# hsinnan75/Dart

Measured on AMD Instinct MI355X. Metric: M paired-end reads/sec (2x101 bp vs GRCh38-sized index), host to host; records bit-identical to CPU dart, higher is better.
Workload: dtype u64/u8 integer

## Files before the change

### dart_amd/csrc/dg_api.hip

```cpp
#include "../../include/dartgpu.h"
#include "dg_common.h"
#include "dg_fm.h"
#include "dg_seedq.h"
#include "dg_chain.h"
#include "dg_report.h"
#include "dg_pair.h"
#include "dg_reseed.h"
#include "dg_sort.h"
#include "dg_samfmt.h"
#include "dg_bamfmt.h"
#include "dg_bgzf.h"
#include "dg_bgzf_dyn.h"
#include "dg_fastq.h"
#include "dg_trim.h"
#include "dg_inflate.h"
#include "dg_sjtab.h"
#include "dg_bamsort.h"
#include "dg_bamidx.h"
#include "dg_coverage.h"
#include "dg_markdup.h"
#include "dg_umidup.h"
#include "dg_pileup.h"
#include "dg_qc.h"
#include "dg_tags.h"
#include "dg_genecount.h"
#include "dg_rnametrics.h"
#include "dg_txquant.h"
#include <stdio.h>
#include <stdlib.h>
#include <string.h>
#include <string>
#include <algorithm>
#include <vector>
#include <atomic>
#include <mutex>
#include <chrono>
#include <thread>
#include <condition_variable>
#include <fcntl.h>
#include <unistd.h>
#include <sys/stat.h>

static char g_init_error[512] = "";

#define DG_HW_QUEUES_NEED 16
static_assert(DG_HW_QUEUES_NEED <= 32, "more hardware queues than 32 are not asked for");
static char g_hwq_found[24] = "unset";
static int g_hwq_left = DG_HW_QUEUES_NEED;
__attribute__((constructor)) static void dg_default_hw_queues()
{
    const char *v = getenv("GPU_MAX_HW_QUEUES");
    long have = 0;
    if (v) {
        size_t i = 0;
        for (; v[i] && i + 1 < sizeof g_hwq_found; i++) g_hwq_found[i] = (v[i] > ' ' && v[i] < 127 && v[i] != ';' && v[i] != '=') ? v[i] : '?';
        g_hwq_found[i] = 0;
        if (!i) snprintf(g_hwq_found, sizeof g_hwq_found, "empty");
        char *end = nullptr;
        have = strtol(v, &end, 10);
        if (end == v || *end) have = 0; else if (have > 1000000) have = 1000000;
    }
    if (have < DG_HW_QUEUES_NEED) {
        char b[8];
        snprintf(b, sizeof b, "%d", DG_HW_QUEUES_NEED);
        setenv("GPU_MAX_HW_QUEUES", b, 1);
        have = DG_HW_QUEUES_NEED;
    }
    g_hwq_left = (int)have;
}
static std::atomic<int> g_live_ctx[64];
static std::atomic<bool> g_hwq_warned{false};

#include "api_ctx.h"

#define N_TIMERS 20
#define N_TOPS 128
enum { TOP_CIG = 0, TOP_SJ, TOP_JOBS, TOP_REPORT_MAIN, TOP_REPORT_JOBS , TOP_HEAVY_UNITS, TOP_SEED_NEXT, TOP_SEED_HEAVY,
       TOP_WORK = 16, TOP_TICKET_PAIR = 17, TOP_TICKET_EMIT = 18, TOP_RESEED_COUNT = 19 , TOP_RESEED_TICKET = 23 , TOP_TICKET_SEED = 26, TOP_RS_POOL = 27, TOP_RS_OUT = 31,
       TOP_ORDER_INFO = 28 , TOP_CLASS_HIST = 32 , TOP_CLASS_FILL = 64  };

struct IndexShared {
    std::mutex mu;
    std::condition_variable cv;
    DIndex ix{};
    std::atomic<uint32_t> gen{1};
    std::thread aids;
    std::atomic<int> aids_state{0};
    char aids_msg[256] = "";
    bool upload_done = false, upload_ok = false;
    void *d_ktab = nullptr, *d_sa_dense = nullptr;
    std::string report, report_out;
    int device = 0;
    uint32_t *d_chr_name_off = nullptr; char *d_chr_names = nullptr; bool chr_names_set = false; uint64_t chr_names_gen = 0; uint32_t chr_name_max = 0;
    uint32_t *d_gc_chr_first = nullptr, *d_gc_seg_start = nullptr, *d_gc_seg_lab = nullptr; uint32_t gc_n_genes = 0; size_t gc_n_seg = 0; uint64_t gc_gen = 0;
    uint32_t *d_rm_chr_first = nullptr, *d_rm_seg_start = nullptr, *d_rm_seg_cs = nullptr; RmTx *d_rm_tx = nullptr; RmExon *d_rm_ex = nullptr;
    size_t rm_n_seg = 0, rm_n_tx = 0, rm_n_elig = 0; uint64_t rm_gen = 0;
    uint32_t *d_tx_chr_first = nullptr, *d_tx_seg_start = nullptr, *d_tx_seg_ids = nullptr; uint64_t *d_tx_seg_off = nullptr; TxTx *d_tx_tx = nullptr; TxExon *d_tx_ex = nullptr;
    size_t tx_n_seg = 0; uint32_t tx_n_tx = 0; uint64_t tx_gen = 0;
};

struct dg_ctx {
    int device = 0;
    IndexShared *shared_ix = nullptr; uint32_t ix_gen = 0;
    bool owns_index = true;
    hipStream_t stream = nullptr;
    hipEvent_t ev_dl = nullptr, ev_dl_block = nullptr;
    bool dl_on_copy_stream = false;
    int env_copy_stream = 1;
    hipEvent_t ev_wait = nullptr;
    char err[512] = "";
    DIndex ix{};
    DParams pr{};
    void *d_bwt = nullptr, *d_sa = nullptr, *d_pac = nullptr, *d_lockey = nullptr, *d_locchr = nullptr, *d_chroff = nullptr;
    int n_reads = 0, max_rlen = 0;
    size_t seq_bytes = 0;
    bool enc_ready = false;
    DBuf<unsigned char> seq; DBuf<uint32_t> seq_off; DBuf<uint16_t> rlen; DBuf<uint32_t> enc; DBuf<uint32_t> packed_in, nlist_in;
    DBuf<DHit> hits; DBuf<uint32_t> nhits, nseeds, seed_off, ncand, rep_off, tile_sums, tile_read, slow_units;
    DBuf<SKey> seeds; DBuf<DSeed> work; DBuf<DCand> cands; DBuf<DJob> jobs; DBuf<unsigned long long> job_items, job_pool; DBuf<RsChunkOut> job_outs; DBuf<uint32_t> job_pool_next; DBuf<unsigned long long> items; DBuf<uint32_t> hist, heavy; DBuf<DHeavy> seed_heavy; DBuf<int32_t> seed_heavy_sfail; DBuf<int16_t> chain_picks; DBuf<uint8_t> chain_todo;
    DBuf<dg_read_out> reads_out; DBuf<dg_report_out> reports; DBuf<uint32_t> cigpool, cigfinal;
    DBuf<dg_sj_out> sjpool, sjfinal;
    DBuf<dg_read_c> reads_c; DBuf<dg_report_c> reports_c; DBuf<uint32_t> cig_c;
    DBuf<unsigned char> ws;
    DBuf<unsigned long long> scan_state, scan_trace;
    int wall_khz = 100000;
    uint32_t scan_epoch = 0;
    size_t cap_seeds = 0, cap_rep = 0, cap_work = 0, cap_cig = 0;
    struct SharedCaps { std::atomic<size_t> seeds{0}, rep{0}, work{0}, cig{0}; } *shared_caps = nullptr;
    bool owns_shared_caps = false;
    unsigned long long *d_ctr = nullptr; unsigned int *d_tops = nullptr; int *d_err = nullptr; DSizes *d_sizes = nullptr; unsigned int *d_input_bad = nullptr;
    struct HostTail { DSizes sizes; int err; unsigned int input_bad; unsigned int tops[N_TOPS]; unsigned long long ctr[CTR_STRIDE]; __host__ __device__ uint32_t *sizes_words() { return (uint32_t *)&sizes; } } *h_tail = nullptr;
    bool state_zeroed = false;
    size_t used[3] = {0, 0, 0};
    bool enqueued = false;
    hipEvent_t ev[N_TIMERS + 1] = {}; const char *tname[N_TIMERS]; int n_t = 0; float tms[N_TIMERS];
    uint64_t counters[CTR_N];
    uint64_t reruns_capacity = 0, reruns_scan = 0;
    bool want_compact = true, packed_valid = false;
    bool batch_done = false;
    bool no_batch = false;
    SamState sam; FqState fq; TrimState tr; InfState inf; BamState bam; SjState sj; BsState bs; BiState bi; CvState cv; MdState md; UdState ud; PuState pu; QcState qc; TgState tg; GcState gc; RmState rm; TxState tx;
    bool want_full = true, full_valid = false;
    int n_cu = 256, runs_of_last_batch = 0, attempt_no = 0;
    int env_seed_waves = 4, env_bail_trips = 0 , env_report_bpc = 8, env_no_fast = 0, env_seed_legacy = 0, env_seed_slots_lg = 0, env_seed_wgs = 0, env_blocking_sync = 0;
    int env_seed_phases = 0, env_seed_wg_waves = 4, env_seed_partial = 32, env_seed_multi = 4;
    bool seed_qf_used = false;
    int env_scan_mask = 7;
    int env_chain_bpc = 8, env_seedh_bpc = 8, env_reseed_pct = 100;
    int env_rs_chunk = RS_CHUNK_DIAGS, env_rs_inline = RS_ENT_INLINE, env_rs_pool = 0;
    int env_scan_budget = 0;
    ~dg_ctx() {
        for (void *p : {(void *)d_ctr, (void *)d_tops, (void *)d_err, (void *)d_sizes, (void *)d_input_bad}) if (p) (void)hipFree(p);
        if (h_tail) (void)hipHostFree(h_tail);
        for (hipEvent_t e : ev) if (e) (void)hipEventDestroy(e);
        for (hipEvent_t e : {ev_wait, ev_dl, ev_dl_block}) if (e) (void)hipEventDestroy(e);
        if (owns_shared_caps) delete shared_caps;
    }
};

static void read_env(dg_ctx *c)
{
    auto geti = [](const char *k, int dflt) { const char *v = getenv(k); return v ? atoi(v) : dflt; };
    c->env_seed_waves = geti("DG_SEED_WAVES", 4); c->env_bail_trips = geti("DG_SEED_BAIL_TRIPS", 0);
    c->env_seed_legacy = geti("DG_SEED_LEGACY", 0); c->env_seed_slots_lg = geti("DG_SEED_SLOTS_LG", 0); c->env_seed_wgs = geti("DG_SEED_WGS", 0); c->env_blocking_sync = geti("DG_BLOCKING_SYNC", 0);
    c->env_report_bpc = geti("DG_REPORT_BPC", 8); c->env_no_fast = geti("DG_NO_FAST_PAIR", 0);
    c->env_scan_budget = geti("DG_SCAN_POLL_BUDGET", 0); c->env_scan_mask = geti("DG_SCAN_POLL_SCANS", 7);
    c->env_seed_phases = geti("DG_SEED_PHASES", 0); c->env_seed_wg_waves = geti("DG_SEED_WG_WAVES", 4); c->env_seed_partial = geti("DG_SEED_PARTIAL_MIN", 32);
    c->env_copy_stream = geti("DG_COPY_STREAM", 1);
    c->env_chain_bpc = std::max(1, geti("DG_CHAIN_BPC", 8)); c->env_seedh_bpc = std::max(1, geti("DG_SEEDH_BPC", 8)); c->env_reseed_pct = std::max(10, geti("DG_RESEED_PCT", 100));
    c->env_rs_chunk = geti("DG_RS_CHUNK", RS_CHUNK_DIAGS); c->env_rs_chunk = std::min(1 << 24, std::max(RS_SUPER, c->env_rs_chunk / RS_SUPER * RS_SUPER));
    c->env_rs_inline = std::min(RS_ENT_INLINE, std::max(0, geti("DG_RS_ENT_MAX", RS_ENT_INLINE))); c->env_rs_pool = std::max(0, geti("DG_RS_POOL_BLOCKS", 0));
    c->sam.first_cap = (size_t)std::max(0, geti("DG_SAM_TEXT_FIRST_CAP", 0));
    c->bam.first_cap = (size_t)std::max(0, geti("DG_BAM_FIRST_CAP", 0));
    c->bs.first_cap = (size_t)std::max(0, geti("DG_BAMSORT_FIRST_CAP", 0));
    c->md.hash_bits = geti("DG_MARKDUP_HASH_BITS", MD_HASH_BITS); if (c->md.hash_bits < 1 || c->md.hash_bits > MD_HASH_BITS) c->md.hash_bits = MD_HASH_BITS;
    c->qc.max_groups = geti("DG_QC_MAX_GROUPS", QC_GROUPS); if (c->qc.max_groups < 1 || c->qc.max_groups > QC_GROUPS) c->qc.max_groups = QC_GROUPS;
    c->rm.max_groups = geti("DG_RNA_MAX_GROUPS", RM_GROUPS); if (c->rm.max_groups < 1 || c->rm.max_groups > RM_GROUPS) c->rm.max_groups = RM_GROUPS;
    c->tx.hash_bits = geti("DG_TX_HASH_BITS", 64); if (c->tx.hash_bits < 1 || c->tx.hash_bits > 64) c->tx.hash_bits = 64;
    c->env_seed_multi = geti("DG_SEED_MULTI", 4); if (c->env_seed_multi < 0 || c->env_seed_multi > SQF_MULTI_MAX) c->env_seed_multi = SQF_MULTI_MAX;
}

static inline void refresh_index(dg_ctx *c)
{
    IndexShared *sh = c->shared_ix;
    if (sh && c->ix_gen != sh->gen.load(std::memory_order_acquire)) { std::lock_guard<std::mutex> lk(sh->mu); c->ix = sh->ix; c->ix_gen = sh->gen.load(); }
}

static int fail(dg_ctx *c, int code, const char *what, hipError_t e)
{
    snprintf(c ? c->err : g_init_error, 512, "%s: %s", what, e == hipSuccess ? "error" : hipGetErrorString(e));
    return code;
}
#define HIPCHK(call) do { hipError_t _e = (call); if (_e != hipSuccess) return fail(c, DG_ERR_HIP, #call, _e); } while (0)

#define SO_PER 8
__global__ void __launch_bounds__(256)
k_seed_offsets(int n_reads, int paired, const uint32_t *__restrict__ nseeds, uint32_t *__restrict__ seed_off, uint32_t *__restrict__ tile_read, uint32_t n_tile_read,
               uint32_t *__restrict__ heavy_list, unsigned int *n_heavy, uint32_t *total_copy, uint32_t cap, TileScan ts, int *err)
{
    __shared__ unsigned long long s_scan[20];
    __shared__ unsigned int s_tile;
    const unsigned int tile = d_tile_ticket_unless(ts, &s_tile, threadIdx.x == 0 && __hip_atomic_load(err, __ATOMIC_RELAXED, __HIP_MEMORY_SCOPE_AGENT) >= DG_ABORT);
    if (tile == SCAN_LEAVE) return;
    const uint32_t first = tile * (256u * SO_PER) + threadIdx.x * SO_PER;
    uint32_t v[SO_PER], sum = 0;
    if (first + SO_PER <= (uint32_t)n_reads) {
        const uint4 a = *(const uint4 *)(nseeds + first), b = *(const uint4 *)(nseeds + first + 4);
        v[0] = a.x; v[1] = a.y; v[2] = a.z; v[3] = a.w; v[4] = b.x; v[5] = b.y; v[6] = b.z; v[7] = b.w;
    } else {
#pragma unroll
        for (int i = 0; i < SO_PER; i++) v[i] = first + i < (uint32_t)n_reads ? nseeds[first + i] : 0u;
    }
#pragma unroll
    for (int i = 0; i < SO_PER; i++) sum += v[i];
    Triple mine, tot;
    mine.x = sum; mine.y = 0; mine.z = 0; mine.w = 0;
    const Triple inb = d_block_exclusive(mine, tot, s_scan);
    const Triple base = d_tile_exclusive(ts, tile, tot, s_scan + 16, err);
    uint32_t run = base.x + inb.x;
    const int lane = threadIdx.x & 63;
#pragma unroll
    for (int i = 0; i < SO_PER; i++) {
        const uint32_t r = first + i;
        if (r < (uint32_t)n_reads) {
            seed_off[r] = run;
            for (uint32_t t = (run + 63u) >> 6; (t << 6) < run + v[i] && t < n_tile_read; t++) tile_read[t] = r;
        }
        const bool unit_end = paired ? (i & 1) == 1 : true;
        const uint32_t useeds = paired ? ((i & 1) ? v[i - ((i & 1) ? 1 : 0)] + v[i] : 0u) : v[i];
        const bool heavy = unit_end && r < (uint32_t)n_reads && useeds > (uint32_t)UNIT_MAX_SEEDS;
        const unsigned long long m = __ballot(heavy);
        if (m) {
            unsigned int hb = 0;
            const int leader = __ffsll((long long)m) - 1;
            if (lane == leader) hb = atomicAdd(n_heavy, (unsigned int)__popcll(m));
            hb = (unsigned int)__shfl((int)hb, leader, 64);
            if (heavy) heavy_list[hb + (unsigned int)__popcll(m & ((1ull << lane) - 1ull))] = paired ? r >> 1 : r;
        }
        run += v[i];
    }
    if (tile == gridDim.x - 1 && threadIdx.x == 0) {
        const uint32_t total = base.x + tot.x;
        seed_off[n_reads] = total;
        if (total_copy) *total_copy = total;
        if (total > cap) atomicMax(err, DG_E_SEEDS);
    }
}

static std::atomic<uint64_t> g_phase_ns[4];
static void caps_publish(std::atomic<size_t> &a, size_t v) { size_t cur = a.load(); while (cur < v && !a.compare_exchange_weak(cur, v)) { } }
static void caps_adopt(size_t &mine, const std::atomic<size_t> &a) { const size_t v = a.load(); if (v > mine) mine = v; }
static std::mutex g_copy_mu[64];
static hipStream_t g_copy_stream[64][2];
static hipError_t copy_stream(int device, int dir, hipStream_t *out)
{
    hipStream_t &sl = g_copy_stream[device & 63][dir];
    if (!sl) {
        int lo = 0, hi = 0;
        hipError_t e = hipDeviceGetStreamPriorityRange(&lo, &hi);
        if (e == hipSuccess) e = hipStreamCreateWithPriority(&sl, hipStreamNonBlocking, hi);
        if (e != hipSuccess) { sl = nullptr; return e; }
    }
    *out = sl;
    return hipSuccess;
}

static bool host_page_locked(const void *p)
{
    if (!p) return false;
    hipPointerAttribute_t a;
    if (hipPointerGetAttributes(&a, p) != hipSuccess) { (void)hipGetLastError(); return false; }
    return a.type == hipMemoryTypeHost;
}

static hipError_t wait_stream(dg_ctx *c)
{
    if (!c->env_blocking_sync || !c->ev_wait) return hipStreamSynchronize(c->stream);
    const hipError_t e = hipEventRecord(c->ev_wait, c->stream);
    return e != hipSuccess ? e : hipEventSynchronize(c->ev_wait);
}

#ifdef DG_PROFILE_CLASSES
__device__ unsigned long long g_class_cycles[DG_COST_CLASSES + 1], g_class_chunks[DG_COST_CLASSES + 1];
#endif
template <int MINW>
__global__ void __launch_bounds__(64, MINW)
k_report(const DIndex ix, const DParams pr, int n_reads, int paired, const unsigned char *__restrict__ seq,
         const uint32_t *__restrict__ seq_off, const uint16_t *__restrict__ rlen, const uint32_t *__restrict__ seed_off,
         const DJob *__restrict__ jobs, DCand *__restrict__ cands,
         const uint32_t *__restrict__ rep_off, DSeed *__restrict__ work, const unsigned long long *__restrict__ items,
         const uint32_t *__restrict__ n_items_p, dg_report_out *__restrict__ reports, uint32_t *cigpool, uint32_t cigcap,
         unsigned int *tops, unsigned char *ws, const WSLayout L, unsigned long long *ctr, int *err)
{
    const unsigned long long t_wave0 = wall_clock64();
    const int lane = blockIdx.x * blockDim.x + threadIdx.x;
    __shared__ uint32_t lds_pm[64 * PM_LDS_WORDS];
    if (*err >= DG_ABORT) return;
    LaneCtx cx;
#ifdef DG_PROFILE_CLASSES
    __shared__ unsigned long long ph_acc[DG_NCLS * DG_NPHASE], cls_acc[2 * DG_NCLS];
    for (int q = threadIdx.x; q < DG_NCLS * DG_NPHASE; q += 64) ph_acc[q] = 0;
    for (int q = threadIdx.x; q < 2 * DG_NCLS; q += 64) cls_acc[q] = 0;
    __syncthreads();
    cx.ph = ph_acc;
#endif
    cx.lds = lds_pm + (threadIdx.x & 63) * PM_LDS_WORDS;
    cx.ix = &ix; cx.pr = &pr; cx.L = &L;
    cx.ws = ws + (size_t)lane * L.stride;
    cx.n_nw = cx.nw_cells = cx.n_reseed = cx.reseed_w = 0;
    const unsigned int lo = 0u, hi = *n_items_p;
    unsigned int *next = tops + TOP_REPORT_MAIN;
    while (true) {
        unsigned int ticket = 0;
        if ((threadIdx.x & 63) == 0) ticket = atomicAdd(next, 1u);
        ticket = (unsigned int)__shfl((int)ticket, 0, 64);
        const unsigned int base = lo + ticket * 64u;
        if (base >= hi) break;
        const unsigned int idx = base + (threadIdx.x & 63);
        const bool valid = idx < hi;
        const unsigned long long item = valid ? items[idx] : 0ull;
        const int r = (int)(item >> 32);
        const uint32_t ci = (uint32_t)item, rep_i = valid ? rep_off[r] + (ci - seed_off[r]) : 0u;
        DRead rd;
        rd.sub_score = 0; rd.mis_num = 0; rd.mapq = 0;
        cx.seq = seq + seq_off[r]; cx.rlen = rlen[r];
#ifdef DG_PROFILE_CLASSES
        const long long t_begin = clock64();
        cx.cls = (int)(cands[(uint32_t)items[base]].final_n & 31); cx.t_last = t_begin;
#endif
        d_gen_mapping_report(cx, valid, paired ? (r & 1) == 0 : true, rd, cands + ci, valid ? 1 : 0, jobs, work,
                             reports + rep_i, rep_i, cigpool, tops + 0, cigcap, err, 0, 1, true);
#ifdef DG_PROFILE_CLASSES
        if ((threadIdx.x & 63) == 0) { cls_acc[cx.cls] += (unsigned long long)(clock64() - t_begin); cls_acc[DG_NCLS + cx.cls] += 1ull; }
#endif
    }
#ifdef DG_PROFILE_CLASSES
    __syncthreads();
    for (int q = threadIdx.x; q < DG_NCLS * DG_NPHASE; q += 64) if (ph_acc[q]) atomicAdd(&g_phase[q / DG_NPHASE][q % DG_NPHASE], ph_acc[q]);
    if (threadIdx.x < DG_NCLS && cls_acc[DG_NCLS + threadIdx.x]) { atomicAdd(&g_class_cycles[threadIdx.x], cls_acc[threadIdx.x]); atomicAdd(&g_class_chunks[threadIdx.x], cls_acc[DG_NCLS + threadIdx.x]); }
#endif
    d_wave_add(ctr + CTR_NW, cx.n_nw);
    d_wave_add(ctr + CTR_NWCELLS, cx.nw_cells);
    d_wave_add(ctr + CTR_RESEED, cx.n_reseed);
    d_wave_add(ctr + CTR_RESEEDW, cx.reseed_w);
    d_wave_resident(ctr, CTR_WT_REPORT, t_wave0);
}

__global__ void __launch_bounds__(256)
k_finalize(const DIndex ix, const DParams pr, int paired, const uint32_t *__restrict__ slow_units, const DSizes *__restrict__ sizes,
           const uint32_t *__restrict__ seed_off, const DCand *__restrict__ cands, const uint32_t *__restrict__ ncand, const uint32_t *__restrict__ rep_off, const DSeed *__restrict__ work,
           dg_read_out *__restrict__ rout, dg_report_out *__restrict__ reports, dg_sj_out *sjpool, uint32_t sjcap, unsigned int *tops, int *err)
{
    if (*err >= DG_ABORT) return;
    const unsigned int n_units = sizes->n_slow_units;
    for (unsigned int it = blockIdx.x * blockDim.x + threadIdx.x; it < n_units; it += gridDim.x * blockDim.x) {
        const int u = (int)slow_units[it];
        const int nm = paired ? 2 : 1;
        DRead rd[2];
        dg_read_out o[2];
        RepMem<dg_report_out> rp[2];
        for (int m = 0; m < nm; m++) {
            const int r = paired ? 2 * u + m : u;
            const int nc = (int)ncand[r];
            dg_report_out *rep = reports + rep_off[r];
            rd[m].score = 0; rd[m].sub_score = 0; rd[m].mis_num = 0; rd[m].mapq = 0; rd[m].iBest = 0; rd[m].CanNum = nc > 0 ? nc : 1;
            for (int i = 0; i < nc; i++) {
                const int aln = rep[i].aln_score, mis_num = rep[i].flag;
                if (mis_num) rep[i].flag = 0;
                if (aln <= 0) continue;
                if (aln > rd[m].score) { rd[m].iBest = i; rd[m].mis_num = mis_num; rd[m].sub_score = rd[m].score; rd[m].score = aln; }
                else if (aln == rd[m].score) rd[m].sub_score = rd[m].score;
            }
            o[m].score = rd[m].score; o[m].sub_score = rd[m].sub_score; o[m].mis_num = rd[m].mis_num; o[m].mapq = 0;
            o[m].n_rep = rd[m].CanNum; o[m].best = rd[m].iBest; o[m].rep_off = (int32_t)rep_off[r]; o[m].sj_off = 0; o[m].n_sj = 0;
            rp[m].p = rep;
        }
        if (paired) {
            d_settle_pair(pr, rd[0], rp[0], rd[1], rp[1]);
            d_flag_pair(rd[0], rp[0], rd[1], rp[1]);
        } else d_flag_single(rd[0], rp[0]);
        for (int m = 0; m < nm; m++) {
            const int r = paired ? 2 * u + m : u;
            d_mapq(rd[m], rp[m]);
            o[m].score = rd[m].score; o[m].mapq = rd[m].mapq; o[m].best = rd[m].iBest;
            if (ncand[r] > 0 && (rd[m].mapq == 50 || (pr.all_sj && rd[m].score > 0)))
                d_collect_sj(ix, pr, cands[seed_off[r] + rd[m].iBest], work, r, sjpool, tops + TOP_SJ, sjcap, o[m].sj_off, o[m].n_sj, err);
            rout[r] = o[m];
        }
    }
}

__global__ void __launch_bounds__(256)
k_emit_slow(int paired, const uint32_t *__restrict__ slow_units, DSizes *sizes, dg_read_out *__restrict__ rout, dg_report_out *__restrict__ reports,
            const uint32_t *__restrict__ cigpool, uint32_t *__restrict__ cigfinal, uint32_t cap_cig, const dg_sj_out *__restrict__ sjpool, dg_sj_out *__restrict__ sjfinal,
            TileScan ts, int *err, const uint16_t *__restrict__ rlen, const CompactOut co)
{
    __shared__ unsigned long long s_scan[20];
    __shared__ unsigned int s_tile;
    bool leave = false;
    if (threadIdx.x == 0) { const int e0 = __hip_atomic_load(err, __ATOMIC_RELAXED, __HIP_MEMORY_SCOPE_AGENT); leave = e0 >= DG_ABORT && e0 != DG_E_CIGFINAL; }
    const unsigned int tile = d_tile_ticket_unless(ts, &s_tile, leave);
    if (tile == SCAN_LEAVE) return;
    const unsigned int n_items = sizes->n_slow_units * (paired ? 2u : 1u);
    if (tile > 0 && tile * 256u >= n_items) return;
    const unsigned int it = tile * 256u + threadIdx.x;
    const bool on = it < n_items;
    const int r = on ? (paired ? (int)(2u * slow_units[it >> 1] + (it & 1u)) : (int)slow_units[it]) : 0;
    dg_read_out o;
    o.n_rep = 0; o.rep_off = 0; o.n_sj = 0; o.sj_off = 0;
    if (on) o = rout[r];
    uint32_t ncig = 0, ncigc = 0;
    const uint32_t full_match = on ? (uint32_t)rlen[r] << 4 : 0u;
    for (int i = 0; i < (on ? o.n_rep : 0); i++) {
        const dg_report_out &rp = reports[o.rep_off + i];
        ncig += rp.n_cigar;
        if (co.reads) ncigc += (rp.n_cigar == 1u && cigpool[rp.cigar_off] == full_match) ? 0u : rp.n_cigar;
    }
    Triple mine, tot;
    mine.x = ncig; mine.y = on ? (uint32_t)o.n_sj : 0u; mine.z = 0; mine.w = ncigc;
    const Triple inb = d_block_exclusive(mine, tot, s_scan);
    const Triple base = d_tile_exclusive(ts, tile, tot, s_scan + 16, err);
    const uint32_t cig_fast = sizes->cig_fast, cigc_fast = sizes->pad[2];
    if (on) {
        uint32_t dst = cig_fast + base.x + inb.x, dstc = cigc_fast + base.w + inb.w;
        bool fits = true;
        if ((uint64_t)dst + ncig > cap_cig) atomicMax(err, DG_E_CIGFINAL);
        else for (int i = 0; i < o.n_rep; i++) {
            dg_report_out &rp = reports[o.rep_off + i];
            const uint32_t m = rp.n_cigar, src = rp.cigar_off;
            const bool plain = m == 1u && cigpool[src] == full_match;
            for (uint32_t k = 0; k < m; k++) cigfinal[dst + k] = cigpool[src + k];
            if (co.reads) {
                if (!plain) { for (uint32_t k = 0; k < m; k++) co.cigar[dstc + k] = cigpool[src + k]; dstc += m; }
                dg_report_c q; fits = d_compact_report(rp, plain, true, q) && fits; co.reports[o.rep_off + i] = q;
            }
            rp.cigar_off = dst; dst += m;
        }
        if (o.n_sj > 0) {
            const uint32_t sd = base.y + inb.y;
            for (int k = 0; k < o.n_sj; k++) sjfinal[sd + k] = sjpool[o.sj_off + k];
            rout[r].sj_off = (int32_t)sd;
        }
        if (co.reads) { dg_read_c oc; fits = d_compact_read(o, oc) && fits; co.reads[r] = oc; if (!fits) *co.bad = 1u; }
    }
    const unsigned int last = n_items ? (n_items - 1u) / 256u : 0u;
    if (tile == last && threadIdx.x == 0) { sizes->total_cig = cig_fast + base.x + tot.x; sizes->total_sj = base.y + tot.y; sizes->pad[0] = cigc_fast + base.w + tot.w; }
}

extern "C" void dg_params_default(dg_params *p)
{
    p->max_gaps = 5; p->max_dup = 100; p->max_intron = 500000; p->min_intron = 5;
    p->max_mismatch = 0; p->multi_hit = 0; p->all_sj = 0; p->paired = 0;
}

static void set_params(dg_ctx *c, const dg_params *p)
{
    c->pr.max_gaps = p->max_gaps; c->pr.max_dup = p->max_dup; c->pr.max_intron = p->max_intron; c->pr.min_intron = p->min_intron;
    c->pr.max_mismatch = p->max_mismatch; c->pr.multi_hit = p->multi_hit; c->pr.all_sj = p->all_sj; c->pr.paired = p->paired;
}

extern "C" int dg_set_params(dg_ctx *c, const dg_params *p)
{
    if (!c || !p) return DG_ERR_ARG;
    set_params(c, p);
    read_env(c);
    return DG_OK;
}

extern "C" int dg_device_count(void)
{
// ... 602 lines not shown
    if (trimmed) {
        const TrimInfo &ti = *c->tr.info.h;
        memcpy(c->tr.stats, ti.stats, sizeof c->tr.stats); c->tr.ms = c->tr.ev.ms(0, 1);
        n_reads = ti.n_kept;
        if (n_reads_out) *n_reads_out = (int)n_reads;
    }
    if (!keep) return DG_OK;
    c->n_reads = (int)n_reads; c->max_rlen = (int)fi.max_rlen; c->seq_bytes = (size_t)fi.total[0];
    c->fq.hdr_bytes = (size_t)fi.total[1]; c->fq.qual_bytes = (size_t)fi.total[2]; c->fq.valid = true;
    return DG_OK;
}

static void fq_forget_batch(dg_ctx *c)
{
    c->n_reads = 0; c->max_rlen = 0; c->seq_bytes = 0; c->enc_ready = false; c->enqueued = false; c->batch_done = false; c->sj.batch_counted = false; c->gc.batch_counted = false; c->tx.batch_counted = false; c->sam.valid = false; c->bam.valid = false; c->bam.rec_valid = false; c->bam.rec_stored = false; c->fq.valid = false;
    c->fq.hdr_bytes = c->fq.qual_bytes = 0; c->fq.ms = 0.f;
    memset(c->tr.stats, 0, sizeof c->tr.stats); c->tr.ms = 0.f; c->tr.enqueued = false;
    c->no_batch = false; c->inf.valid = false; c->fq.tail_valid = false; c->fq.tail_n[0] = c->fq.tail_n[1] = 0;
}

extern "C" int dg_batch_upload_fastq(dg_ctx *c, const dg_fastq_text *in, int *n_reads_out)
{
    if (!c) return DG_ERR_ARG;
    if (n_reads_out) *n_reads_out = 0;
    fq_forget_batch(c);
    if (!in) { snprintf(c->err, 512, "dg_batch_upload_fastq: the input is NULL"); return DG_ERR_ARG; }
    const size_t n1 = in->text1 ? in->n1 : 0, n2 = in->text2 ? in->n2 : 0;
    const bool two = in->text2 != nullptr && in->n2 > 0;
    if ((in->n1 && !in->text1) || in->max_reads < 0) { snprintf(c->err, 512, "dg_batch_upload_fastq: text1 is NULL or max_reads is negative"); return DG_ERR_ARG; }
    if (n1 >= 0xFFFFFF00ull || n2 >= 0xFFFFFF00ull) { snprintf(c->err, 512, "dg_batch_upload_fastq: a text must be smaller than 2^32 - 256 bytes"); return DG_ERR_ARG; }
    if (n1 == 0 && !two) { c->fq.valid = true; return DG_OK; }
    HIPCHK(hipSetDevice(c->device));
    FqPlan p;
    p.n[0] = n1; p.n[1] = n2; p.two = two; p.max_reads = (size_t)in->max_reads;
    { const int rc = fq_reserve(c, p); if (rc) return rc; }
    if (n1) HIPCHK(hipMemcpyAsync(c->fq.text.p, in->text1, n1, hipMemcpyHostToDevice, c->stream));
    if (n2) HIPCHK(hipMemcpyAsync(c->fq.text.p + p.off2, in->text2, n2, hipMemcpyHostToDevice, c->stream));
    HIPCHK(hipEventRecord(c->fq.ev[0], c->stream));
    { const int rc = fq_enqueue(c, p, in->rc_odd_reads, false, false, true); if (rc) return rc; }
    HIPCHK(wait_stream(c));
    return fq_finish(c, "dg_batch_upload_fastq", in->max_reads, n_reads_out, true);
}

static int inf_enqueue_copies(dg_ctx *c, const std::vector<InfBlock> &tab, const void *src1, size_t n1, const void *src2, size_t n2, size_t in_off2)
{
    HIPCHK(c->inf.in.ensure(std::max(n1, in_off2 + n2) + 8)); HIPCHK(c->inf.tab.ensure(tab.size() + 1)); HIPCHK(c->inf.status.ensure(tab.size() + 1));
    if (n1) HIPCHK(hipMemcpyAsync(c->inf.in.p, src1, n1, hipMemcpyHostToDevice, c->stream));
    if (n2) HIPCHK(hipMemcpyAsync(c->inf.in.p + in_off2, src2, n2, hipMemcpyHostToDevice, c->stream));
    if (!tab.empty()) HIPCHK(hipMemcpyAsync(c->inf.tab.p, tab.data(), tab.size() * sizeof(InfBlock), hipMemcpyHostToDevice, c->stream));
    HIPCHK(hipMemsetAsync(c->inf.verdict.d, 0xff, 8, c->stream));
    return DG_OK;
}
static int inf_enqueue_kernel(dg_ctx *c, size_t n_blocks, unsigned char *d_out)
{
    if (n_blocks) k_bgzf_inflate<<<(unsigned)((n_blocks + INF_WAVES - 1) / INF_WAVES), 64 * INF_WAVES, 0, c->stream>>>(c->inf.in.p, c->inf.tab.p, (uint32_t)n_blocks, d_out, c->inf.status.p, c->inf.verdict.d);
    HIPCHK(hipGetLastError());
    HIPCHK(c->inf.verdict.fetch(c->stream));
    return DG_OK;
}

extern "C" int dg_inflate_granules(int out[2])
{
    if (!out) return DG_ERR_ARG;
    out[0] = INF_WAVES; out[1] = (int)INF_ROUND;
    return DG_OK;
}

extern "C" int dg_bgzf_inflate(dg_ctx *c, const void *host_bytes, size_t n, size_t *n_out, size_t *n_blocks, float *device_ms)
{
    if (!c) return DG_ERR_ARG;
    if (n_out) *n_out = 0;
    if (n_blocks) *n_blocks = 0;
    if (device_ms) *device_ms = 0.f;
    c->inf.valid = false; c->inf.bytes = 0;
    if (n == 0) { c->inf.valid = true; return DG_OK; }
    if (!host_bytes) { snprintf(c->err, 512, "dg_bgzf_inflate: the input is NULL"); return DG_ERR_ARG; }
    std::vector<InfBlock> tab;
    size_t total = 0, bad = 0;
    if (const char *why = inf_walk_members((const unsigned char *)host_bytes, n, 0, 0, tab, &total, &bad)) { snprintf(c->err, 512, "dg_bgzf_inflate: block %zu: %s", bad, why); return DG_ERR_ARG; }
    if (tab.size() > 0x7fffffffull) { snprintf(c->err, 512, "dg_bgzf_inflate: %zu blocks are more than one call takes", tab.size()); return DG_ERR_ARG; }
    HIPCHK(hipSetDevice(c->device));
    HIPCHK(c->inf.ready());
    HIPCHK(c->inf.out.ensure(total + 32));
    { const int rc = inf_enqueue_copies(c, tab, host_bytes, n, nullptr, 0, 0); if (rc) return rc; }
    HIPCHK(hipEventRecord(c->inf.ev[0], c->stream));
    { const int rc = inf_enqueue_kernel(c, tab.size(), c->inf.out.p); if (rc) return rc; }
    HIPCHK(hipEventRecord(c->inf.ev[1], c->stream));
    HIPCHK(wait_stream(c));
    const float ms = c->inf.ev.ms(0, 1);
    if (device_ms) *device_ms = ms;
    if (n_blocks) *n_blocks = tab.size();
    const unsigned long long v = *c->inf.verdict.h;
    if (v != ~0ull) { snprintf(c->err, 512, "dg_bgzf_inflate: block %llu: %s", v >> 8, inf_rule((uint32_t)(v & 0xffu))); return DG_ERR_ARG; }
    c->inf.valid = true; c->inf.bytes = total;
    if (n_out) *n_out = total;
    return DG_OK;
}

extern "C" int dg_inflate_download(dg_ctx *c, void *out, size_t cap)
{
    if (!c) return DG_ERR_ARG;
    if (!c->inf.valid) { snprintf(c->err, 512, "dg_inflate_download: no inflated bytes (dg_bgzf_inflate first)"); return DG_ERR_ARG; }
    if (cap < c->inf.bytes) { snprintf(c->err, 512, "dg_inflate_download: output capacity too small: %zu bytes of %zu", cap, c->inf.bytes); return DG_ERR_CAPACITY; }
    if (c->inf.bytes == 0) return DG_OK;
    if (!out) return DG_ERR_ARG;
    HIPCHK(hipSetDevice(c->device));
    HIPCHK(hipMemcpyAsync(out, c->inf.out.p, c->inf.bytes, hipMemcpyDeviceToHost, c->stream));
    HIPCHK(wait_stream(c));
    return DG_OK;
}

extern "C" int dg_inflate_device(dg_ctx *c, void **ptr, size_t *n_out)
{
    if (!c || !ptr || !n_out) return DG_ERR_ARG;
    if (!c->inf.valid) { snprintf(c->err, 512, "dg_inflate_device: no inflated bytes (dg_bgzf_inflate first)"); return DG_ERR_ARG; }
    *ptr = c->inf.bytes ? c->inf.out.p : nullptr; *n_out = c->inf.bytes;
    return DG_OK;
}

extern "C" int dg_batch_upload_fastq_bgzf(dg_ctx *c, const dg_fastq_bgzf *in, uint32_t flags, int *n_reads_out, size_t tail[2], uint64_t *n_unlike)
{
    static const char *fn = "dg_batch_upload_fastq_bgzf";
    if (!c) return DG_ERR_ARG;
    if (n_reads_out) *n_reads_out = 0;
    if (tail) tail[0] = tail[1] = 0;
    if (n_unlike) *n_unlike = 0;
    fq_forget_batch(c);
    if (!in) { snprintf(c->err, 512, "%s: the input is NULL", fn); return DG_ERR_ARG; }
    if (flags & ~DG_FQ_CHECK_ONLY) { snprintf(c->err, 512, "%s: unknown flag bits 0x%x", fn, flags & ~DG_FQ_CHECK_ONLY); return DG_ERR_ARG; }
    const bool check_only = (flags & DG_FQ_CHECK_ONLY) != 0, two = in->blocks2 != nullptr || in->head2 != nullptr, last = in->last != 0;
    if ((in->n_head1 && !in->head1) || (in->n_blocks1 && !in->blocks1) || (in->n_head2 && !in->head2) || (in->n_blocks2 && !in->blocks2) || in->max_reads < 0) {
        snprintf(c->err, 512, "%s: a length without its pointer, or max_reads is negative", fn); return DG_ERR_ARG;
    }
    const size_t nh[2] = { in->head1 ? in->n_head1 : 0, in->head2 ? in->n_head2 : 0 }, nb[2] = { in->blocks1 ? in->n_blocks1 : 0, two && in->blocks2 ? in->n_blocks2 : 0 };
    const unsigned char *src[2] = { (const unsigned char *)in->blocks1, (const unsigned char *)in->blocks2 };
    const size_t in_off2 = (nb[0] + 255) & ~(size_t)255;
    std::vector<InfBlock> tab;
    size_t n_inf[2] = {0, 0}, first2 = 0;
    for (int f = 0; f < (two ? 2 : 1); f++) {
        size_t bad = 0;
        if (f) first2 = tab.size();
        if (const char *why = inf_walk_members(src[f], nb[f], f ? in_off2 : 0, nh[f], tab, &n_inf[f], &bad)) { snprintf(c->err, 512, "%s: text %d block %zu: %s", fn, f + 1, bad, why); return DG_ERR_ARG; }
        if (nh[f] + n_inf[f] >= 0xFFFFFF00ull) { snprintf(c->err, 512, "%s: a text must be smaller than 2^32 - 256 bytes", fn); return DG_ERR_ARG; }
    }
    if (!two) first2 = tab.size();
    if (tab.size() > 0x7fffffffull) { snprintf(c->err, 512, "%s: %zu blocks are more than one call takes", fn, tab.size()); return DG_ERR_ARG; }
    FqPlan p;
    p.n[0] = nh[0] + n_inf[0]; p.n[1] = nh[1] + n_inf[1]; p.two = two; p.max_reads = (size_t)in->max_reads;
    if (p.n[0] == 0 && p.n[1] == 0) { c->fq.valid = !check_only; c->no_batch = check_only; c->fq.tail_valid = true; return DG_OK; }
    HIPCHK(hipSetDevice(c->device));
    HIPCHK(c->inf.ready());
    { const int rc = fq_reserve(c, p); if (rc) return rc; }
    for (size_t k = first2; k < tab.size(); k++) tab[k].out_off += p.off2;
    c->fq.tail_off2 = (p.n[0] + 255) & ~(size_t)255;
    HIPCHK(c->fq.tail.ensure(c->fq.tail_off2 + p.n[1] + 16));
    { const int rc = inf_enqueue_copies(c, tab, src[0], nb[0], src[1], nb[1], in_off2); if (rc) return rc; }
    if (nh[0]) HIPCHK(hipMemcpyAsync(c->fq.text.p, in->head1, nh[0], hipMemcpyHostToDevice, c->stream));
    if (nh[1]) HIPCHK(hipMemcpyAsync(c->fq.text.p + p.off2, in->head2, nh[1], hipMemcpyHostToDevice, c->stream));
    HIPCHK(hipEventRecord(c->fq.ev[0], c->stream));
    { const int rc = inf_enqueue_kernel(c, tab.size(), c->fq.text.p); if (rc) return rc; }
    { const int rc = fq_enqueue(c, p, in->rc_odd_reads, !last, true, !check_only); if (rc) return rc; }
    HIPCHK(wait_stream(c));
    const unsigned long long v = *c->inf.verdict.h;
    if (v != ~0ull) {
        const size_t k = (size_t)(v >> 8);
        snprintf(c->err, 512, "%s: text %d block %zu: %s", fn, k >= first2 ? 2 : 1, k >= first2 ? k - first2 : k, inf_rule((uint32_t)(v & 0xffu)));
        return DG_ERR_ARG;
    }
    const FqInfo &fi = *c->fq.info.h;
    if (n_unlike) *n_unlike = fi.n_unlike;
    const int rc = fq_finish(c, fn, in->max_reads, n_reads_out, !check_only);
    if (fi.status == FQ_OK || fi.status == FQ_E_EMPTY || fi.status == FQ_E_LONG || fi.status == FQ_E_OFFSETS) {
        c->fq.tail_n[0] = p.n[0] - fi.tail_at[0]; c->fq.tail_n[1] = two ? p.n[1] - fi.tail_at[1] : 0;
        c->fq.tail_valid = true;
        if (tail) { tail[0] = c->fq.tail_n[0]; tail[1] = c->fq.tail_n[1]; }
    }
    if (rc == DG_OK && check_only) c->no_batch = true;
    return rc;
}

extern "C" int dg_batch_download_fastq_tail(dg_ctx *c, char *tail1, size_t cap1, char *tail2, size_t cap2)
{
    if (!c) return DG_ERR_ARG;
    if (!c->fq.tail_valid) { snprintf(c->err, 512, "dg_batch_download_fastq_tail: no tails (dg_batch_upload_fastq_bgzf first)"); return DG_ERR_ARG; }
    if (cap1 < c->fq.tail_n[0] || cap2 < c->fq.tail_n[1]) { snprintf(c->err, 512, "dg_batch_download_fastq_tail: output capacity too small (need %zu %zu)", c->fq.tail_n[0], c->fq.tail_n[1]); return DG_ERR_CAPACITY; }
    if ((c->fq.tail_n[0] && !tail1) || (c->fq.tail_n[1] && !tail2)) return DG_ERR_ARG;
    if (!c->fq.tail_n[0] && !c->fq.tail_n[1]) return DG_OK;
    HIPCHK(hipSetDevice(c->device));
    if (c->fq.tail_n[0]) HIPCHK(hipMemcpyAsync(tail1, c->fq.tail.p, c->fq.tail_n[0], hipMemcpyDeviceToHost, c->stream));
    if (c->fq.tail_n[1]) HIPCHK(hipMemcpyAsync(tail2, c->fq.tail.p + c->fq.tail_off2, c->fq.tail_n[1], hipMemcpyDeviceToHost, c->stream));
    HIPCHK(wait_stream(c));
    return DG_OK;
}

extern "C" int dg_batch_fastq_device_ms(dg_ctx *c, float *ms)
{
    if (!c || !ms) return DG_ERR_ARG;
    *ms = c->fq.ms;
    return DG_OK;
}

extern "C" int dg_set_trim(dg_ctx *c, const dg_trim *t)
{
    if (!c) return DG_ERR_ARG;
    if (!t) { c->tr.on = false; return DG_OK; }
    if (t->flags & ~DG_TRIM_PAIRS) { snprintf(c->err, 512, "dg_set_trim: unknown flag bits 0x%x", t->flags & ~DG_TRIM_PAIRS); return DG_ERR_ARG; }
    if (t->min_len == 0 || t->min_overlap == 0) { snprintf(c->err, 512, "dg_set_trim: min_len and min_overlap must be at least 1"); return DG_ERR_ARG; }
    if (t->max_err_permille > 1000u) { snprintf(c->err, 512, "dg_set_trim: max_err_permille is %u, above 1000", t->max_err_permille); return DG_ERR_ARG; }
    if (t->poly_mask & ~15u) { snprintf(c->err, 512, "dg_set_trim: poly_mask 0x%x has a bit above 3", t->poly_mask); return DG_ERR_ARG; }
    if (t->qual3 > TR_QUAL_MAX || t->qual5 > TR_QUAL_MAX || t->qual_base > TR_QUAL_MAX) { snprintf(c->err, 512, "dg_set_trim: qual3, qual5 and qual_base must not exceed %u", TR_QUAL_MAX); return DG_ERR_ARG; }
    TrimPar par = {};
    for (int i = 0; i < 2; i++) {
        if (t->n_adapter[i] > 64u) { snprintf(c->err, 512, "dg_set_trim: adapter %d has %u bases, more than 64", i, t->n_adapter[i]); return DG_ERR_ARG; }
        for (uint32_t j = 0; j < t->n_adapter[i]; j++) {
            const char b = t->adapter[i][j];
            if (b != 'A' && b != 'C' && b != 'G' && b != 'T') { snprintf(c->err, 512, "dg_set_trim: adapter %d has a byte outside ACGT at %u", i, j); return DG_ERR_ARG; }
            par.acode[i][j >> 5] |= (uint64_t)trim_code(b) << (2u * (j & 31u));
        }
        par.alen[i] = t->n_adapter[i];
    }
    par.flags = t->flags; par.qual3 = t->qual3; par.qual5 = t->qual5; par.qual_base = t->qual_base; par.min_overlap = t->min_overlap; par.max_err_permille = t->max_err_permille;
    par.poly_mask = t->poly_mask; par.poly_min = t->poly_min; par.min_len = t->min_len;
    c->tr.par = par; c->tr.on = true;
    return DG_OK;
}

extern "C" int dg_set_umi(dg_ctx *c, const dg_umi *u)
{
    if (!c) return DG_ERR_ARG;
    if (!u) { c->tr.umi_on = false; return DG_OK; }
    if (u->flags & ~DG_UMI_PAIRS) { snprintf(c->err, 512, "dg_set_umi: unknown flag bits 0x%x", u->flags & ~DG_UMI_PAIRS); return DG_ERR_ARG; }
    if ((uint64_t)u->len[0] + u->len[1] == 0 || (uint64_t)u->len[0] + u->len[1] > UD_MAX_LEN) { snprintf(c->err, 512, "dg_set_umi: the two lengths together are %llu, not 1..%d", (unsigned long long)u->len[0] + u->len[1], UD_MAX_LEN); return DG_ERR_ARG; }
    for (int m = 0; m < 2; m++)
        if ((uint64_t)u->len[m] + u->skip[m] > (uint64_t)DG_MAX_RLEN) { snprintf(c->err, 512, "dg_set_umi: len[%d] + skip[%d] is %llu, above %d", m, m, (unsigned long long)u->len[m] + u->skip[m], DG_MAX_RLEN); return DG_ERR_ARG; }
    if (u->sep == 0 || u->sep == ' ' || u->sep == '\t' || u->sep == '/' || ud_code((unsigned char)u->sep)) { snprintf(c->err, 512, "dg_set_umi: the separator 0x%02x is NUL, a blank, a tab, '/' or one of ACGTN+-", (unsigned char)u->sep); return DG_ERR_ARG; }
    c->tr.umi = *u; c->tr.umi_on = true;
    return DG_OK;
}

extern "C" int dg_batch_trim_stats(dg_ctx *c, uint64_t stats[16], float *device_ms)
{
    if (!c || !stats) return DG_ERR_ARG;
    memcpy(stats, c->tr.stats, sizeof c->tr.stats);
    if (device_ms) *device_ms = c->tr.ms;
    return DG_OK;
}

extern "C" int dg_trim_granules(int out[2])
{
    if (!out) return DG_ERR_ARG;
    out[0] = FQ_THREADS; out[1] = 64;
    return DG_OK;
}

extern "C" int dg_batch_download_reads(dg_ctx *c, uint32_t *seq_off, uint16_t *rlen, char *seq, uint32_t *hdr_off, char *hdr, uint32_t *qual_off, char *qual,
                                       const size_t caps[3], size_t used[3])
{
    if (!c || !caps || !used) return DG_ERR_ARG;
    if (!c->fq.valid) { snprintf(c->err, 512, "dg_batch_download_reads: the context's last upload was not dg_batch_upload_fastq"); return DG_ERR_ARG; }
    used[0] = c->seq_bytes; used[1] = c->fq.hdr_bytes; used[2] = c->fq.qual_bytes;
    if (caps[0] < used[0] || caps[1] < used[1] || caps[2] < used[2]) { snprintf(c->err, 512, "dg_batch_download_reads: output capacity too small (need %zu %zu %zu)", used[0], used[1], used[2]); return DG_ERR_CAPACITY; }
    const size_t n = (size_t)c->n_reads;
    if (n == 0) { if (hdr_off) hdr_off[0] = 0; if (qual_off) qual_off[0] = 0; return DG_OK; }
    if (!seq_off || !rlen || !hdr_off || !qual_off || (used[0] && !seq) || (used[1] && !hdr) || (used[2] && !qual)) return DG_ERR_ARG;
    HIPCHK(hipSetDevice(c->device));
    HIPCHK(hipMemcpyAsync(seq_off, c->seq_off.p, n * 4, hipMemcpyDeviceToHost, c->stream));
    HIPCHK(hipMemcpyAsync(rlen, c->rlen.p, n * 2, hipMemcpyDeviceToHost, c->stream));
    HIPCHK(hipMemcpyAsync(hdr_off, c->fq.hdr_off.p, (n + 1) * 4, hipMemcpyDeviceToHost, c->stream));
    HIPCHK(hipMemcpyAsync(qual_off, c->fq.qual_off.p, (n + 1) * 4, hipMemcpyDeviceToHost, c->stream));
    if (used[0]) HIPCHK(hipMemcpyAsync(seq, c->seq.p, used[0], hipMemcpyDeviceToHost, c->stream));
    if (used[1]) HIPCHK(hipMemcpyAsync(hdr, c->fq.hdr.p, used[1], hipMemcpyDeviceToHost, c->stream));
    if (used[2]) HIPCHK(hipMemcpyAsync(qual, c->fq.qual.p, used[2], hipMemcpyDeviceToHost, c->stream));
    HIPCHK(wait_stream(c));
    return DG_OK;
}

extern "C" void *dg_host_alloc(size_t bytes)
{
    void *p = nullptr;
    return hipHostMalloc(&p, bytes ? bytes : 1, hipHostMallocDefault) == hipSuccess ? p : nullptr;
}
extern "C" void dg_host_free(void *p) { if (p) (void)hipHostFree(p); }

static WSLayout make_ws_layout(int R)
{
    WSLayout L;
    auto al = [](uint32_t x) { return (x + 15u) & ~15u; };
    uint32_t o = 0;
    const uint32_t nmax = 2u * (uint32_t)R + 32u;
    L.max_rlen = (uint32_t)R;
    L.cig_off = o; L.cig_cap = 4u * (uint32_t)R + 64u; o = al(o + L.cig_cap * 4u);
    L.nwbits_off = o; L.nwbits_words = ((uint32_t)R + 1u) * ((nmax + 7u) / 8u); o = al(o + L.nwbits_words * 4u);
    L.rows_off = o; L.row_cap = (uint32_t)R + 8u; o = al(o + 2u * L.row_cap * 4u);
    L.str_off = o; L.str_cap = al(3u * (uint32_t)R + 64u); o = al(o + 6u * L.str_cap);
    L.kmer_off = o; L.kmer_cap = (uint32_t)R + 8u > 48u ? (uint32_t)R + 8u : 48u; o = al(o + L.kmer_cap * 8u);
    uint32_t rd = 64; while (rd < (uint32_t)R + 1u) rd <<= 1;
    L.ring_diag = rd; L.ring_words = ((uint32_t)R + 64u) / 64u; L.ring_off = o; o = al(o + rd * L.ring_words * 8u);
    L.stride = (o + 255u) & ~255u;
    return L;
}

#define DG_MAX_DEVICES 64
static std::mutex g_lds_mu;
static size_t g_lds_set[2][DG_MAX_DEVICES];
static hipError_t raise_dynamic_lds(const void *fn, int which, int device, size_t lds)
{
    std::lock_guard<std::mutex> lk(g_lds_mu);
    size_t &cur = g_lds_set[which][device & (DG_MAX_DEVICES - 1)];
    if (lds <= cur) return hipSuccess;
    const hipError_t e = hipFuncSetAttribute(fn, hipFuncAttributeMaxDynamicSharedMemorySize, (int)lds);
    if (e == hipSuccess) cur = lds;
    return e;
}

static hipError_t launch_seed(dg_ctx *c, int n, int H, hipEvent_t after_encode = nullptr)
{
    const int W = 2 * ((c->max_rlen + 15) / 16 > 0 ? (c->max_rlen + 15) / 16 : 1);
    hipError_t e = c->enc.ensure((size_t)W * n + 16);
    if (e != hipSuccess) return e;
    int lg = 0;
    while ((1 << lg) < W / 2) lg++;
    if (!c->enc_ready) k_encode<<<(unsigned)((((size_t)n << lg) + 255) / 256), 256, 0, c->stream>>>(c->seq.p, c->seq_off.p, c->rlen.p, n, W, lg, c->enc.p);
    if (after_encode) { e = hipEventRecord(after_encode, c->stream); if (e != hipSuccess) return e; }
    if ((e = c->seed_heavy.ensure((size_t)n + 16)) != hipSuccess) return e;
    unsigned blocks = (unsigned)c->n_cu * (unsigned)c->env_seed_waves;
    if ((size_t)blocks * 64 > (size_t)n) blocks = (unsigned)((n + 63) / 64);
    const bool use_qf = !c->env_seed_legacy && !c->env_seed_phases && W <= 62 && c->pr.max_dup <= 30000;
    const int bail_trips = c->env_bail_trips > 0 ? c->env_bail_trips : (use_qf ? 64 : 128);
    unsigned int *tops = c->d_tops;
    c->seed_qf_used = false;
    if (use_qf) {
        int lg = c->env_seed_slots_lg >= 6 && c->env_seed_slots_lg <= 11 ? c->env_seed_slots_lg : 9;
        int nw = c->env_seed_wg_waves >= 1 && c->env_seed_wg_waves <= 8 ? c->env_seed_wg_waves : 4;
        while (lg > 6 && sqf_lds_bytes(lg, W, nw) > (size_t)156 * 1024) lg--;
        if (c->env_seed_slots_lg == 0) while (lg > 6 && sqf_lds_bytes(lg, W, nw) > (size_t)80 * 1024) lg--;
        const size_t lds = sqf_lds_bytes(lg, W, nw);
        if ((e = raise_dynamic_lds((const void *)k_seed_qf, 0, c->device, lds)) != hipSuccess) return e;
        unsigned per_cu = (unsigned)(((size_t)160 * 1024) / lds);
        if (per_cu * (unsigned)nw > 16u) per_cu = 16u / (unsigned)nw;
        if (per_cu > 2u) per_cu = 2u;
        if (per_cu < 1u) per_cu = 1u;
        if (c->env_seed_wgs > 0) per_cu = (unsigned)c->env_seed_wgs;
        unsigned wgs = (unsigned)c->n_cu * per_cu;
        const unsigned need = (unsigned)(((size_t)n + ((size_t)1 << lg) - 1) >> lg);
        if (wgs > need) wgs = need;
        c->seed_qf_used = true;
        k_seed_qf<<<wgs, nw * 64, lds, c->stream>>>(c->ix, c->pr, c->enc.p, c->rlen.p, n, W, H, lg, c->hits.p, c->nhits.p, c->nseeds.p, tops + TOP_SEED_NEXT,
                                                    c->seed_heavy.p, tops + TOP_SEED_HEAVY, c->d_ctr, bail_trips, c->env_seed_partial, c->env_seed_multi, c->d_err, bail_trips);
    } else
    if (!c->env_seed_legacy && W <= 62) {
        int lg = c->env_seed_slots_lg >= 6 && c->env_seed_slots_lg <= 10 ? c->env_seed_slots_lg : 9;
        while (lg > 6 && sq_lds_bytes(lg, W) > (size_t)80 * 1024) lg--;
        const size_t lds = sq_lds_bytes(lg, W);
        if ((e = raise_dynamic_lds((const void *)k_seed_q, 1, c->device, lds)) != hipSuccess) return e;
        unsigned per_cu = (unsigned)(((size_t)160 * 1024) / lds);
        if (per_cu > 4u) per_cu = 4u;
        if (c->env_seed_wgs > 0) per_cu = (unsigned)c->env_seed_wgs;
        unsigned wgs = (unsigned)c->n_cu * per_cu;
        const unsigned need = (unsigned)(((size_t)n + ((size_t)1 << lg) - 1) >> lg);
        if (wgs > need) wgs = need;
        k_seed_q<<<wgs, SQ_THREADS, lds, c->stream>>>(c->ix, c->pr, c->enc.p, c->rlen.p, n, W, H, lg, c->hits.p, c->nhits.p, c->nseeds.p, tops + TOP_SEED_NEXT,
                                                      c->seed_heavy.p, tops + TOP_SEED_HEAVY, c->d_ctr, bail_trips, c->d_err);
    } else
    if (W <= 78) k_seed<true><<<blocks, 64, ((size_t)2 * W * 64 + 64) * 4, c->stream>>>(c->ix, c->pr, c->enc.p, c->rlen.p, n, W, H, c->hits.p, c->nhits.p, c->nseeds.p, tops + TOP_SEED_NEXT, c->seed_heavy.p, tops + TOP_SEED_HEAVY, c->d_ctr, bail_trips);
    else k_seed<false><<<blocks, 64, 0, c->stream>>>(c->ix, c->pr, c->enc.p, c->rlen.p, n, W, H, c->hits.p, c->nhits.p, c->nseeds.p, tops + TOP_SEED_NEXT, c->seed_heavy.p, tops + TOP_SEED_HEAVY, c->d_ctr, bail_trips);
    if ((e = c->seed_heavy_sfail.ensure((size_t)n + 16)) != hipSuccess) return e;
    k_seed_heavy_walk<<<(unsigned)c->n_cu * 8u, 64, 0, c->stream>>>(c->ix, c->pr, c->enc.p, c->rlen.p, W, c->seed_heavy.p, tops + TOP_SEED_HEAVY, c->seed_heavy_sfail.p, c->d_ctr);
    k_seed_heavy<<<(unsigned)c->n_cu * (unsigned)c->env_seedh_bpc, 64, (size_t)W * 4 + 16, c->stream>>>(c->ix, c->pr, c->enc.p, c->rlen.p, W, H, c->hits.p, c->nhits.p, c->nseeds.p, c->seed_heavy.p, tops + TOP_SEED_HEAVY, c->seed_heavy_sfail.p, c->d_ctr);
    return hipGetLastError();
}

static TileScan make_tile_scan(dg_ctx *c, size_t first_tile, unsigned int *ticket, int which )
{
    TileScan ts;
    ts.w = c->scan_state.p + SCAN_WORDS * first_tile; ts.ticket = ticket; ts.epoch = c->scan_epoch;
    ts.budget = (c->env_scan_budget > 0 && c->attempt_no == 0 && (c->env_scan_mask & which)) ? (uint32_t)c->env_scan_budget : 0u;
    ts.dbg = c->d_sizes->scan_dbg;
    ts.ticks = (unsigned long long)c->wall_khz * 2000ull;
    ts.trace = c->scan_trace.p ? c->scan_trace.p + SCAN_TRACE_WORDS * first_tile : nullptr;
    return ts;
}

#define TICK(name) do { if (c->n_t < N_TIMERS) { c->tname[c->n_t] = name; HIPCHK(hipEventRecord(c->ev[c->n_t + 1], c->stream)); c->n_t++; } } while (0)

static int enqueue_seeding(dg_ctx *c, int n, int H, bool timed, bool paired_units)
{
    HIPCHK(c->hits.ensure((size_t)n * H)); HIPCHK(c->nhits.ensure(n)); HIPCHK(c->nseeds.ensure(n)); HIPCHK(c->seed_off.ensure((size_t)n + 1));
    if (c->shared_caps) caps_adopt(c->cap_seeds, c->shared_caps->seeds);
    if (c->cap_seeds < (size_t)n * 3 + 1024) c->cap_seeds = (size_t)n * 3 + 1024;
    HIPCHK(c->seeds.ensure(c->cap_seeds + 1)); HIPCHK(c->cands.ensure(c->cap_seeds + 1)); HIPCHK(c->tile_read.ensure(c->cap_seeds / 64 + 16));
    if (timed) c->tname[c->n_t] = "k_encode";
    HIPCHK(launch_seed(c, n, H, timed ? c->ev[c->n_t + 1] : nullptr));
    if (timed) { c->n_t++; TICK("k_seed"); }
    {
        const int paired = (paired_units && (n % 2 == 0)) ? 1 : 0;
        HIPCHK(c->heavy.ensure((size_t)n + 16));
        const TileScan ts_seed = make_tile_scan(c, 0, c->d_tops + TOP_TICKET_SEED, 1);
        k_seed_offsets<<<(unsigned)((n + 256 * SO_PER - 1) / (256 * SO_PER)), 256, 0, c->stream>>>(n, paired, c->nseeds.p, c->seed_off.p, c->tile_read.p, (uint32_t)c->tile_read.cap,
                                                                                                 c->heavy.p, c->d_tops + TOP_HEAVY_UNITS, &c->d_sizes->total_seeds, (uint32_t)c->cap_seeds, ts_seed, c->d_err);
        HIPCHK(hipGetLastError());
    }
    if (timed) TICK("seed_offsets");
    k_locate<<<(unsigned)((c->cap_seeds + 255) / 256), 256, 0, c->stream>>>(c->ix, n, H, c->hits.p, c->tile_read.p, c->seed_off.p, c->seeds.p, c->d_ctr, c->d_err);
    HIPCHK(hipGetLastError());
    if (timed) TICK("k_locate");
    return DG_OK;
}

__global__ void __launch_bounds__(256)
k_batch_begin(unsigned long long *ctr, unsigned int *tops, int *err, DSizes *sizes)
{
    for (int i = threadIdx.x; i < CTR_STRIPES * CTR_STRIDE; i += 256) ctr[i] = 0ull;
    if (threadIdx.x < N_TOPS) tops[threadIdx.x] = 0u;
    if (threadIdx.x < (int)(sizeof(DSizes) / 4)) ((uint32_t *)sizes)[threadIdx.x] = 0u;
    if (threadIdx.x == 0) *err = 0;
}

static size_t scan_tiles_seed(int n_reads) { return (size_t)(n_reads + 256 * SO_PER - 1) / (256 * SO_PER) + 1; }
static size_t scan_tiles_pair(int n_units) { return (size_t)(n_units + PU_THREADS - 1) / PU_THREADS + 1; }

__global__ void __launch_bounds__(256)
k_batch_end(DSizes *__restrict__ sizes, int *__restrict__ err, unsigned int *__restrict__ tops, unsigned long long *__restrict__ ctr, dg_ctx::HostTail *out)
{
    const int t = threadIdx.x;
    if (t < (int)(sizeof(DSizes) / 4)) { out->sizes_words()[t] = ((const uint32_t *)sizes)[t]; ((uint32_t *)sizes)[t] = 0u; }
    if (t < N_TOPS) { out->tops[t] = tops[t]; tops[t] = 0u; }
    if (t == 0) { out->err = *err; *err = 0; }
    if (t < CTR_STRIDE) {
        const bool is_max = t == CTR_MAXTRIPS || t == CTR_WTRIPS_MAX;
        unsigned long long v = 0;
        for (int s_ = 0; s_ < CTR_STRIPES; s_++) { const unsigned long long x = ctr[s_ * CTR_STRIDE + t]; ctr[s_ * CTR_STRIDE + t] = 0ull; v = is_max ? (x > v ? x : v) : v + x; }
        out->ctr[t] = v;
    }
}

static int zero_batch_state(dg_ctx *c, int n_reads, int n_units)
{
    if (!c->state_zeroed) {
        k_batch_begin<<<1, 256, 0, c->stream>>>(c->d_ctr, c->d_tops, c->d_err, c->d_sizes);
        HIPCHK(hipGetLastError());
    }
    c->state_zeroed = false;
    const size_t tiles2 = (size_t)(2 * n_units + 255) / 256 + 1;
    const size_t words = SCAN_WORDS * (scan_tiles_seed(n_reads) + scan_tiles_pair(n_units) + tiles2);
    if (words > c->scan_state.cap) {
        HIPCHK(c->scan_state.ensure(words));
        HIPCHK(hipMemsetAsync(c->scan_state.p, 0, c->scan_state.cap * 8, c->stream));
        static_assert(SCAN_TRACE_WORDS == SCAN_WORDS, "the trace array is sized like the state array");
        HIPCHK(c->scan_trace.ensure(c->scan_state.cap));
        HIPCHK(hipMemsetAsync(c->scan_trace.p, 0, c->scan_trace.cap * 8, c->stream));
    }
    c->scan_epoch = (c->scan_epoch + 1u) & 0x3FFFFFFFu;
    if (c->scan_epoch == 0) c->scan_epoch = 1;
    return DG_OK;
}


static int enqueue_run(dg_ctx *c)
{
    const int n = c->n_reads;
    const int paired = (c->pr.paired && (n % 2 == 0)) ? 1 : 0;
    const int n_units = paired ? n / 2 : n;
    refresh_index(c);
    c->n_t = 0;
    const int H = c->max_rlen / 16 + 1;
    const uint32_t nb = (uint32_t)((n + 255) / 256);
    { const int zr = zero_batch_state(c, n, n_units); if (zr) return zr; }
    HIPCHK(hipEventRecord(c->ev[0], c->stream));
    { const int rc = enqueue_seeding(c, n, H, true, c->pr.paired != 0); if (rc) return rc; }

    if (c->shared_caps) { caps_adopt(c->cap_rep, c->shared_caps->rep); caps_adopt(c->cap_cig, c->shared_caps->cig); caps_adopt(c->cap_work, c->shared_caps->work); }
    if (c->cap_rep < (size_t)n + (size_t)n / 4 + 1024) c->cap_rep = (size_t)n + (size_t)n / 4 + 1024;
    if (c->cap_cig < 3 * c->cap_rep) c->cap_cig = 3 * c->cap_rep;
    if (c->cap_work < (size_t)n * 8 + 65536) c->cap_work = (size_t)n * 8 + 65536;
    const size_t cigcap = (size_t)n * 48 + c->cap_rep * (16 + CIG_SLOT) + 4096, sjcap = (size_t)n * 4 + 1024;
    HIPCHK(c->ncand.ensure(n)); HIPCHK(c->rep_off.ensure((size_t)n + 1)); HIPCHK(c->reads_out.ensure(n));
    HIPCHK(c->heavy.ensure((size_t)n_units + 16)); HIPCHK(c->slow_units.ensure((size_t)n_units + 16));
    HIPCHK(c->reports.ensure(c->cap_rep + 1)); HIPCHK(c->work.ensure(c->cap_work + 16)); HIPCHK(c->jobs.ensure(c->cap_seeds + 16));
    const uint32_t rs_out_cap = (uint32_t)std::max<size_t>(16384, (size_t)n / 8), rs_list_cap = (uint32_t)std::min<size_t>(c->jobs.cap + rs_out_cap, 0xFFFFFFF0u);
    HIPCHK(c->job_outs.ensure(rs_out_cap)); HIPCHK(c->job_items.ensure(3 * (size_t)rs_list_cap + 16));
    const uint32_t rs_pool_cap = (uint32_t)std::max<size_t>(16384, (size_t)n / 32);
    HIPCHK(c->job_pool.ensure((size_t)rs_pool_cap * 64)); HIPCHK(c->job_pool_next.ensure(rs_pool_cap));
    HIPCHK(c->cigpool.ensure(cigcap)); HIPCHK(c->cigfinal.ensure(c->cap_cig + 16)); HIPCHK(c->sjpool.ensure(sjcap)); HIPCHK(c->sjfinal.ensure(sjcap));
    HIPCHK(c->items.ensure(c->cap_seeds + 16));
    unsigned int *tops = c->d_tops;

    HIPCHK(c->chain_picks.ensure(c->cap_seeds + 16)); HIPCHK(c->chain_todo.ensure((size_t)n_units + 16));
    k_chain_heavy<<<c->n_cu * c->env_chain_bpc, 64, 0, c->stream>>>(c->ix, c->pr, n_units, paired, c->rlen.p, c->seed_off.p, c->seeds.p, c->cands.p, c->ncand.p,
                                                     c->heavy.p, tops + TOP_HEAVY_UNITS, c->chain_picks.p, c->chain_todo.p, c->d_ctr, c->d_err);
    k_chain_rules<<<c->n_cu * 4, 64, 0, c->stream>>>(paired, c->seed_off.p, c->cands.p, c->ncand.p, c->heavy.p, tops + TOP_HEAVY_UNITS, c->chain_picks.p, c->chain_todo.p, c->d_err);
    HIPCHK(hipGetLastError());
#ifdef DG_PROFILE_CLASSES
    {
        unsigned long long v[3], z = 0;
        HIPCHK(hipStreamSynchronize(c->stream));
        HIPCHK(hipMemcpyFromSymbol(&v[0], HIP_SYMBOL(g_chain_max), 8)); HIPCHK(hipMemcpyFromSymbol(&v[1], HIP_SYMBOL(g_chain_units), 8)); HIPCHK(hipMemcpyFromSymbol(&v[2], HIP_SYMBOL(g_chain_cycles), 8));
        HIPCHK(hipMemcpyToSymbol(HIP_SYMBOL(g_chain_max), &z, 8)); HIPCHK(hipMemcpyToSymbol(HIP_SYMBOL(g_chain_units), &z, 8)); HIPCHK(hipMemcpyToSymbol(HIP_SYMBOL(g_chain_cycles), &z, 8));
        fprintf(stderr, "[chain_heavy] units %llu  mean cycles %llu  max cycles %llu (seeds %llu/%llu cands %llu/%llu)\n", v[1], v[1] ? v[2] / v[1] : 0, v[0] >> 40,
                (v[0] >> 30) & 1023, (v[0] >> 20) & 1023, (v[0] >> 10) & 1023, v[0] & 1023);
    }
#endif
    TICK("k_chain_heavy");
    const size_t tiles_s = scan_tiles_seed(n), tiles = scan_tiles_pair(n_units);
    const TileScan ts_pair = make_tile_scan(c, tiles_s, tops + TOP_TICKET_PAIR, 2), ts_emit = make_tile_scan(c, tiles_s + tiles, tops + TOP_TICKET_EMIT, 4);
    const int try_fast = (c->env_no_fast || c->ix.n_chr > 0xFFFF) ? 0 : 1;
    CompactOut co{nullptr, nullptr, nullptr, nullptr};
    if (c->want_compact) {
        HIPCHK(c->reads_c.ensure((size_t)n + 1)); HIPCHK(c->reports_c.ensure(c->cap_rep + 1)); HIPCHK(c->cig_c.ensure(c->cap_cig + 16));
        co = CompactOut{c->reads_c.p, c->reports_c.p, c->cig_c.p, &c->d_sizes->pad[1]};
    }
    const int W2p = (c->max_rlen + 15) / 16 > 0 ? (c->max_rlen + 15) / 16 : 1;
    const bool packed_pair = c->enc_ready;
    auto launch_pair = [&](auto kernel) {
        kernel<<<(unsigned)((n_units + PU_THREADS - 1) / PU_THREADS), PU_THREADS, 0, c->stream>>>(
            c->ix, c->pr, n_units, paired, try_fast, (c->want_full || !c->want_compact) ? 0 : 2, c->seq.p, c->seq_off.p, c->enc.p, W2p, c->rlen.p, c->seed_off.p, c->seeds.p, c->cands.p, c->ncand.p, c->rep_off.p,
            c->slow_units.p, c->reads_out.p, c->reports.p, c->cigfinal.p, (uint32_t)c->cap_rep, (uint32_t)c->cap_cig, ts_pair, c->d_sizes, tops + TOP_CIG, c->d_ctr, c->d_err, co);
    };
    if (packed_pair) launch_pair(k_pair<true>); else launch_pair(k_pair<false>);
    HIPCHK(hipGetLastError());
    TICK("k_pair");

    const WSLayout L = make_ws_layout(c->max_rlen < 32 ? 32 : c->max_rlen);
    int blocks = c->n_cu * c->env_report_bpc;
    if ((size_t)blocks * 64 > (size_t)n) blocks = (n + 63) / 64;
    {
        const size_t budget = (size_t)12 << 30, per_block = (size_t)64 * L.stride;
        if ((size_t)blocks * per_block > budget) blocks = (int)(budget / per_block);
        if (blocks < 1) blocks = 1;
    }
    HIPCHK(c->ws.ensure((size_t)blocks * 64 * L.stride));
    unsigned slow_grid = (unsigned)c->n_cu * 4u;
    if ((size_t)slow_grid * 256 > (size_t)n) slow_grid = nb;
    k_prep<dg_report_out><<<slow_grid, 256, 0, c->stream>>>(c->pr, paired, c->slow_units.p, c->d_sizes, c->seed_off.p, c->seeds.p, c->cands.p, c->ncand.p, c->work.p, tops + TOP_WORK,
                                             (uint32_t)c->cap_work, c->jobs.p, tops + TOP_JOBS, (uint32_t)c->jobs.cap, c->d_err, c->rlen.p, c->rep_off.p, c->reports.p, tops + TOP_CLASS_HIST,
                                             packed_pair ? c->enc.p : nullptr, W2p, c->seq.p);
    HIPCHK(hipGetLastError());
    TICK("k_prep");
    const uint32_t jobcap = (uint32_t)c->jobs.cap;
    const RsPool rs_pool{c->job_pool.p, c->job_pool_next.p, tops + TOP_RS_POOL, c->env_rs_pool > 0 ? std::min<uint32_t>((uint32_t)c->env_rs_pool, rs_pool_cap) : rs_pool_cap};
    const int rs_gap_max = c->max_rlen - 32, rs_need = rs_gap_max >= 8 ? (rs_gap_max - 8) / 64 + 1 : 1;
    const RsOrder rs_order{c->jobs.p, tops + TOP_JOBS, jobcap, c->job_items.p, rs_list_cap, rs_out_cap, rs_need <= 1 ? 1 : (rs_need <= 2 ? 2 : 4), (uint32_t)c->env_rs_chunk, tops + TOP_RESEED_COUNT, tops + TOP_RS_OUT};
    k_order<<<slow_grid, 256, 0, c->stream>>>(paired, c->slow_units.p, c->d_sizes, c->seed_off.p, c->cands.p, c->ncand.p, tops + TOP_CLASS_HIST, tops + TOP_CLASS_FILL, c->items.p, tops + TOP_ORDER_INFO, rs_order, c->d_err);
    HIPCHK(hipGetLastError());
    TICK("order");
    k_reseed<1><<<c->n_cu * 10 * c->env_reseed_pct / 100, 64, 0, c->stream>>>(c->ix, c->seq.p, c->seq_off.p, c->jobs.p, c->job_items.p, tops + TOP_RESEED_COUNT, tops + TOP_RESEED_COUNT + 3, tops + TOP_RESEED_TICKET, c->job_outs.p, rs_pool, c->env_rs_inline, c->d_ctr, c->d_err);
    if (rs_need > 1) k_reseed<2><<<c->n_cu * 6 * c->env_reseed_pct / 100, 64, 0, c->stream>>>(c->ix, c->seq.p, c->seq_off.p, c->jobs.p, c->job_items.p + rs_list_cap, tops + TOP_RESEED_COUNT + 1, tops + TOP_RESEED_COUNT + 3, tops + TOP_RESEED_TICKET + 1, c->job_outs.p, rs_pool, c->env_rs_inline, c->d_ctr, c->d_err);
    if (rs_need > 2) k_reseed<4><<<c->n_cu * 4 * c->env_reseed_pct / 100, 64, 0, c->stream>>>(c->ix, c->seq.p, c->seq_off.p, c->jobs.p, c->job_items.p + 2 * (size_t)rs_list_cap, tops + TOP_RESEED_COUNT + 2, tops + TOP_RESEED_COUNT + 3, tops + TOP_RESEED_TICKET + 2, c->job_outs.p, rs_pool, c->env_rs_inline, c->d_ctr, c->d_err);
    HIPCHK(hipGetLastError());
    TICK("k_reseed");
    const uint32_t *n_items_p = tops + TOP_ORDER_INFO + 1;
    k_report<2><<<blocks, 64, 0, c->stream>>>(c->ix, c->pr, n, paired, c->seq.p, c->seq_off.p, c->rlen.p, c->seed_off.p, c->jobs.p, c->cands.p,
                                               c->rep_off.p, c->work.p, c->items.p, n_items_p, c->reports.p, c->cigpool.p,
                                               (uint32_t)cigcap, tops, c->ws.p, L, c->d_ctr, c->d_err);
    HIPCHK(hipGetLastError());
#ifdef DG_PROFILE_CLASSES
    {
        unsigned long long cyc[DG_COST_CLASSES + 1], cnt[DG_COST_CLASSES + 1], z[DG_COST_CLASSES + 1] = {0};
        HIPCHK(hipStreamSynchronize(c->stream));
        HIPCHK(hipMemcpyFromSymbol(cyc, HIP_SYMBOL(g_class_cycles), sizeof cyc)); HIPCHK(hipMemcpyFromSymbol(cnt, HIP_SYMBOL(g_class_chunks), sizeof cnt));
        HIPCHK(hipMemcpyToSymbol(HIP_SYMBOL(g_class_cycles), z, sizeof z)); HIPCHK(hipMemcpyToSymbol(HIP_SYMBOL(g_class_chunks), z, sizeof z));
        unsigned long long tot = 0; for (int k = 0; k <= DG_COST_CLASSES; k++) tot += cyc[k];
        unsigned long long ph[DG_NCLS][DG_NPHASE], zp[DG_NCLS][DG_NPHASE] = {{0}};
        HIPCHK(hipMemcpyFromSymbol(ph, HIP_SYMBOL(g_phase), sizeof ph)); HIPCHK(hipMemcpyToSymbol(HIP_SYMBOL(g_phase), zp, sizeof zp));
        for (int k = 0; k < DG_COST_CLASSES; k++) if (cnt[k]) {
            fprintf(stderr, "[class %2d] chunks %7llu  cycles/chunk %8llu  share %5.1f %%  phases/chunk:", k, cnt[k], cyc[k] / cnt[k], 100.0 * cyc[k] / (tot ? tot : 1));
            for (int q = 0; q < DG_NPHASE; q++) fprintf(stderr, " %llu", ph[k][q] / cnt[k]);
            fprintf(stderr, "\n");
        }
    }
#endif
    TICK("k_report");
    k_finalize<<<slow_grid, 256, 0, c->stream>>>(c->ix, c->pr, paired, c->slow_units.p, c->d_sizes, c->seed_off.p, c->cands.p, c->ncand.p, c->rep_off.p, c->work.p,
                                                 c->reads_out.p, c->reports.p, c->sjpool.p, (uint32_t)sjcap, tops, c->d_err);
    k_emit_slow<<<(unsigned)((n + 255) / 256), 256, 0, c->stream>>>(paired, c->slow_units.p, c->d_sizes, c->reads_out.p, c->reports.p, c->cigpool.p, c->cigfinal.p,
                                                                    (uint32_t)c->cap_cig, c->sjpool.p, c->sjfinal.p, ts_emit, c->d_err, c->rlen.p, co);
    HIPCHK(hipGetLastError());
    TICK("k_finalize");
    k_batch_end<<<1, 256, 0, c->stream>>>(c->d_sizes, c->d_err, c->d_tops, c->d_ctr, c->h_tail);
    HIPCHK(hipGetLastError());
    c->state_zeroed = true;
    TICK("tail");
    c->enqueued = true;
    return DG_OK;
}

static int finish_run(dg_ctx *c, size_t used[3])
{
    c->runs_of_last_batch = 0;
    for (int attempt = 0; attempt < 6; attempt++) {
        c->runs_of_last_batch++;
        HIPCHK(wait_stream(c));
        if (c->enc_ready && c->h_tail->input_bad) { snprintf(c->err, 512, "packed batch: the N list holds a position outside the batch"); c->enqueued = false; return DG_ERR_ARG; }
        const DSizes &sz = c->h_tail->sizes;
        const int derr = c->h_tail->err;
        if (derr < DG_ABORT) break;
        auto grow = [](size_t need) { return need + need / 4 + 1024; };
        if (derr == DG_E_SEEDS) c->cap_seeds = grow(sz.total_seeds);
        else if (derr == DG_E_REPORTS) {
            c->cap_rep = std::max(grow(sz.total_rep), 2 * c->cap_rep);
            if (c->cap_cig < 3 * c->cap_rep) c->cap_cig = 3 * c->cap_rep;
        }
        else if (derr == DG_E_WORK) c->cap_work = grow(c->h_tail->tops[TOP_WORK]);
        else if (derr == DG_E_CIGFINAL) c->cap_cig = grow(sz.total_cig > 2 * c->cap_cig ? sz.total_cig : 2 * c->cap_cig);
        if (c->shared_caps) { caps_publish(c->shared_caps->seeds, c->cap_seeds); caps_publish(c->shared_caps->rep, c->cap_rep); caps_publish(c->shared_caps->work, c->cap_work); caps_publish(c->shared_caps->cig, c->cap_cig); }
        if (derr == DG_E_SEEDS || derr == DG_E_REPORTS || derr == DG_E_WORK || derr == DG_E_CIGFINAL) {  }
        else if ((derr == DG_E_SCAN || derr == DG_E_SEEDQ) && attempt < 5) {
            c->reruns_scan++;
            const unsigned long long *d = sz.scan_dbg;
            const double tick_ms = 1.0 / (double)c->wall_khz;
            const bool same_epoch = (d[8] >> 32) == d[5];
            snprintf(c->err, 512, "batch run again (device status %d): look-back of tile %llu gave up on tile %lld after %llu polls / %.1f ms (lane %llu, epoch %llu): words %016llx %016llx %016llx; "
                     "stuck tile's trace: epoch %llu%s HW_ID %08llx (wave %llu simd %llu cu %llu sh %llu se %llu) XCC %llu, ticket %.3f ms before the give-up, own totals %s, prefix %s",
                     derr, d[0] ? d[0] - 1 : 0ull, (long long)d[1], d[6], (double)(d[12] - d[13]) * tick_ms, d[7], d[5], d[2], d[3], d[4],
                     d[8] >> 32, same_epoch ? "" : " (NOT this run's: it never took its ticket here)", d[8] & 0xFFFFFFFFull, d[8] & 15, (d[8] >> 4) & 3, (d[8] >> 8) & 15, (d[8] >> 12) & 1, (d[8] >> 13) & 7, d[11] >> 56,
                     (double)(d[12] - d[9]) * tick_ms, d[10] ? "published" : "NOT published", (d[11] & 0x00FFFFFFFFFFFFFFull) ? "published" : "NOT published");
            if (!c->env_scan_budget) fprintf(stderr, "[libdartgpu] %s\n", c->err);
        }
        else { snprintf(c->err, 512, "device-side scan did not complete (status %d)", derr); return DG_ERR_INTERNAL; }
        if (attempt == 5) { snprintf(c->err, 512, "buffer capacities did not converge (status %d)", derr); return DG_ERR_INTERNAL; }
        if (derr != DG_E_SCAN && derr != DG_E_SEEDQ) c->reruns_capacity++;
        c->attempt_no = attempt + 1;
        const int rc = enqueue_run(c);
        if (rc) return rc;
    }
    c->enqueued = false;
    for (int i = 0; i < c->n_t; i++) { float ms = 0; (void)hipEventElapsedTime(&ms, c->ev[i], c->ev[i + 1]); c->tms[i] = ms; }
    static_assert(CTR_N <= CTR_STRIDE, "the work counters fill one stripe");
    for (int k = 0; k < CTR_N; k++) c->counters[k] = c->h_tail->ctr[k];
    if (c->seed_qf_used) {
        c->counters[CTR_STEPS_ACT] += c->counters[CTR_SQ_LANES + SQ_STEP]; c->counters[CTR_BLOCKS_ACT] += c->counters[CTR_SQ_LANES + SQ_STEP];
        c->counters[CTR_KTAB] += c->counters[CTR_SQ_LANES + SQ_BEGIN]; c->counters[CTR_DIRECT] += c->counters[CTR_SQ_LANES + SQ_LOC] + c->counters[CTR_SQ_LANES + SQ_CMP];
    }
    const DSizes &sz = c->h_tail->sizes;
    c->counters[CTR_SEEDS] = sz.total_seeds;
    const int derr = c->h_tail->err;
    if (derr) { snprintf(c->err, 512, "device pool exhausted (%s)", derr == DG_E_CIGAR ? "cigar" : (derr == DG_E_SJ ? "splice junction" : "reseed jobs")); return DG_ERR_INTERNAL; }
    c->used[0] = sz.total_rep; c->used[1] = sz.total_cig; c->used[2] = sz.total_sj;
    c->packed_valid = c->want_compact; c->full_valid = c->want_full || !c->want_compact;
    if (used) { used[0] = c->used[0]; used[1] = c->used[1]; used[2] = c->used[2]; }
    return DG_OK;
}

extern "C" int dg_batch_run(dg_ctx *c, size_t used[3])
{
    if (!c) return DG_ERR_ARG;
    if (c->no_batch) { snprintf(c->err, 512, "dg_batch_run: the context holds no batch (its last upload was a DG_FQ_CHECK_ONLY)"); return DG_ERR_ARG; }
    HIPCHK(hipSetDevice(c->device));
    c->inf.valid = false;
    c->used[0] = c->used[1] = c->used[2] = 0;
    memset(c->counters, 0, sizeof c->counters);
// ... 3207 lines not shown
```

### dart_amd/csrc/dg_seedq.h

```cpp
#pragma once
#include "dg_fm.h"

#define SQ_WAVES   4
#define SQ_THREADS (SQ_WAVES * 64)
enum { SQ_BEGIN = 0, SQ_STEP = 1, SQ_CMP = 2, SQ_LOC = 3, SQ_FREE = 4, SQ_NQ = 5 };
#define SQ_MAX_PHASES (1u << 20)

__device__ __forceinline__ uint32_t sq_rfl(uint32_t v) { return (uint32_t)__builtin_amdgcn_readfirstlane((int)v); }

__host__ __device__ inline size_t sq_lds_bytes(int nslot_lg, int W)
{
    const size_t n = (size_t)1 << nslot_lg;
    return n * 48 + n * 4 * (size_t)W + 2 * n * 2 * SQ_NQ + SQ_WAVES * 64 * 2 + 16 * 4;
}

struct SqEnv {
    const DIndex &ix; const DParams &pr;
    uint4 *st; uint32_t *rd;
    int NSLOT, W2, K, H, bail_trips; bool direct;
    int multi;
    DHit *hits; uint32_t *nhits, *nseeds; DHeavy *heavy; unsigned int *n_heavy;
};

template <int MODE>
__device__ __forceinline__ int sq_trip(const SqEnv &e, const bool act, const uint32_t slot, SeedCtr &c, uint32_t &max_trips)
{
    const DIndex &ix = e.ix;
    const int NSLOT = e.NSLOT, W2 = e.W2;
    uint32_t *rd = e.rd; uint4 *st = e.st;
    int nq = SQ_FREE;
    uint4 A = make_uint4(0, 0, 0, 0), B = A, C = A;
    if (act) { A = st[slot * 3]; if (MODE != SQ_BEGIN) { B = st[slot * 3 + 1]; C = st[slot * 3 + 2]; } }
    const int r = (int)A.x, len = (int)(A.y & 0xFFFFu), end_pos = len - 13;
    int pos = (int)(A.y >> 16), nh = (int)(A.z & 0xFFFu);
    uint32_t nsearch = (A.z >> 12) & 0xFFu, trips = A.z >> 20, ns = A.w;
    Search s;
    s.mode = MODE; s.hit_len = 0; s.located = false;
    s.start = (int)(B.x & 0xFFFFu); s.p = (int)(B.x >> 16); s.ref_steps = B.y & 0xFFFFu; s.ref_blocks = B.y >> 16;
    s.x0 = s.x1 = s.lk = 0; s.x2 = 1; s.tpos = 0; s.lsteps = 0;
    if (MODE == SQ_STEP) { s.x0 = d_u64(B.z, B.w); s.x1 = d_u64(C.x, C.y); s.x2 = d_u64(C.z, C.w); }
    else if (MODE == SQ_LOC) { s.lk = d_u64(B.z, B.w); s.lsteps = C.x; }
    else if (MODE == SQ_CMP) { s.tpos = (int64_t)d_u64(B.z, B.w); s.lk = d_u64(C.x, C.y); s.lsteps = C.z; }
    auto rb = [&](int w) -> uint32_t { const int wc = w < W2 ? w : W2 - 1; const uint32_t v = rd[(size_t)wc * NSLOT + slot]; return w < W2 ? v : 0u; };
    auto rm = [&](int w) -> uint32_t { const int wc = w < W2 ? w : W2 - 1; const uint32_t v = rd[(size_t)(W2 + wc) * NSLOT + slot]; return w < W2 ? v : 0xFFFFFFFFu; };
    bool live = act, finished = false, beginning = false;
    TripData t; t.aux = T_NONE;
    TripAddr ta = {nullptr, nullptr, nullptr, nullptr};
    if (act) {
        trips = trips < 4095u ? trips + 1u : trips;
        if (MODE == SQ_BEGIN) {
            while (pos < end_pos && d_at(rm, pos)) pos++;
            if (pos >= end_pos) finished = true;
            else if (nsearch >= SEED_BAIL || trips >= (uint32_t)e.bail_trips) {
                DHeavy hv; hv.read = (uint32_t)r; hv.pos = pos; hv.nh = nh; hv.ns = ns;
                e.heavy[atomicAdd(e.n_heavy, 1u)] = hv;
                max_trips = trips > max_trips ? trips : max_trips;
                live = false;
            } else { nsearch++; beginning = true; d_begin_issue(ix, e.K, rb, rm, pos, s, c, ta, t); }
        } else d_trip_issue(ix, rm, len, e.direct, s, c, ta, t);
    }
    d_trip_load(ta, t);
    if (live) {
        if (MODE == SQ_BEGIN) { if (beginning) d_begin_finish(ix, e.K, rb, s, c, t); }
        else if (t.aux != T_NONE) d_trip_finish(ix, e.pr, rb, rm, len, s, c, t);
        if (e.direct && s.mode == 1 && s.x2 == 1) { s.mode = 3; s.lk = s.x0; s.lsteps = 0; }
        if (s.mode == 1 && (s.p >= len || d_at(rm, s.p))) d_search_end(e.pr, s);
        if (!finished && s.mode == 0) {
            c.steps += s.ref_steps; c.blocks += s.ref_blocks;
            if (s.hit_len) {
                if (nh < e.H) {
                    DHit h; h.rPos = (uint16_t)s.start; h.len = (uint16_t)s.hit_len;
                    if (s.located) { h.x0 = (uint64_t)s.tpos; h.freq = 1u | 0x80000000u; c.lf_ref += s.lsteps + (uint32_t)(s.lk >> 40); }
                    else { h.x0 = s.x0; h.freq = (uint32_t)s.x2; }
                    e.hits[(size_t)r * e.H + nh] = h;
                }
                nh++; ns += (uint32_t)s.x2;
                pos = s.start + s.hit_len;
            } else pos = s.start + 1;
            while (pos < end_pos && d_at(rm, pos)) pos++;
            if (pos >= end_pos) finished = true;
        }
        if (finished) { e.nhits[r] = (uint32_t)nh; e.nseeds[r] = ns; max_trips = trips > max_trips ? trips : max_trips; }
        else {
            nq = s.mode;
            A.y = (uint32_t)len | ((uint32_t)pos << 16); A.z = (uint32_t)nh | (nsearch << 12) | (trips << 20); A.w = ns;
            B.x = (uint32_t)s.start | ((uint32_t)s.p << 16); B.y = (s.ref_steps & 0xFFFFu) | (s.ref_blocks << 16);
            if (s.mode == 1) { B.z = (uint32_t)s.x0; B.w = (uint32_t)(s.x0 >> 32); C = make_uint4((uint32_t)s.x1, (uint32_t)(s.x1 >> 32), (uint32_t)s.x2, (uint32_t)(s.x2 >> 32)); }
            else if (s.mode == 3) { B.z = (uint32_t)s.lk; B.w = (uint32_t)(s.lk >> 32); C.x = s.lsteps; }
            else if (s.mode == 2) { B.z = (uint32_t)s.tpos; B.w = (uint32_t)((uint64_t)s.tpos >> 32); C.x = (uint32_t)s.lk; C.y = (uint32_t)(s.lk >> 32); C.z = s.lsteps; }
            st[slot * 3] = A;
            if (s.mode != 0) { st[slot * 3 + 1] = B; st[slot * 3 + 2] = C; }
        }
    }
    return nq;
}

__global__ void __launch_bounds__(SQ_THREADS)
k_seed_q(const DIndex ix, const DParams pr, const uint32_t *__restrict__ enc, const uint16_t *__restrict__ rlen, int n_reads, int W, int H, int nslot_lg,
         DHit *__restrict__ hits, uint32_t *__restrict__ nhits, uint32_t *__restrict__ nseeds, unsigned int *next_read,
         DHeavy *__restrict__ heavy, unsigned int *n_heavy, unsigned long long *ctr, int bail_trips, int *err)
{
    extern __shared__ uint4 sq_sh[];
    const int NSLOT = 1 << nslot_lg;
    const int QCAP = 2 * NSLOT;
    const uint32_t SM = (uint32_t)QCAP - 1u;
    uint4 *st = sq_sh;
    uint32_t *rd = (uint32_t *)(st + 3 * (size_t)NSLOT);
    uint16_t *q = (uint16_t *)(rd + (size_t)W * NSLOT);
    uint16_t *tab = q + (size_t)SQ_NQ * QCAP;
    uint32_t *ctl = (uint32_t *)(tab + SQ_WAVES * 64);
    const int tid = threadIdx.x, lane = tid & 63;
    const int wave = (int)sq_rfl((uint32_t)(tid >> 6));
    const int W2 = W >> 1;
    const int K = ix.ktab ? ix.ktab_k : 0;
    const bool direct = ix.sa_dense != nullptr;
    const uint32_t w_magic = ((1u << 20) + (uint32_t)W - 1u) / (uint32_t)W;
    SeedCtr c = {0, 0, 0, 0, 0, 0, 0, 0};
    uint32_t max_trips = 0, wtrips = 0;
    const SqEnv env = { ix, pr, st, rd, NSLOT, W2, K, H, bail_trips, direct, 0, hits, nhits, nseeds, heavy, n_heavy };
    uint32_t q_trips[SQ_NQ] = {0, 0, 0, 0, 0}, q_lanes[SQ_NQ] = {0, 0, 0, 0, 0};

    for (int i = tid; i < NSLOT; i += SQ_THREADS) q[(size_t)SQ_FREE * QCAP + i] = (uint16_t)i;
    if (tid < 16) ctl[tid] = tid == 5 + SQ_FREE ? (uint32_t)NSLOT : 0u;

    uint32_t n_phases = 0;
    for (uint32_t phase = 0; ; phase++) {
        n_phases = phase;
        __syncthreads();
        uint32_t hd[SQ_NQ], cn[SQ_NQ];
#pragma unroll
        for (int k = 0; k < SQ_NQ; k++) { hd[k] = sq_rfl(ctl[k]); cn[k] = sq_rfl(ctl[5 + k]) - hd[k]; }
        const bool ex = sq_rfl(ctl[10]) != 0u;
        __syncthreads();
        if (cn[SQ_FREE] == (uint32_t)NSLOT && ex) break;
        if (phase >= SQ_MAX_PHASES) { if (tid == 0) atomicMax(err, DG_E_SEEDQ); break; }
        const uint32_t f_free = (ex || cn[SQ_FREE] < 64u) ? 0u : 1u;
        const uint32_t r_free = (ex || cn[SQ_FREE] >= 64u) ? 0u : cn[SQ_FREE];
        const uint32_t p0 = f_free, p1 = p0 + (cn[SQ_CMP] >> 6), p2 = p1 + (cn[SQ_LOC] >> 6), p3 = p2 + (cn[SQ_STEP] >> 6), p4 = p3 + (cn[SQ_BEGIN] >> 6);
        int my_q = SQ_BEGIN;
        uint32_t my_n = 0, my_first = 0;
        const uint32_t wv = (uint32_t)wave;
        if (wv < p4) {
            my_n = 64u;
            if (wv < p0) { my_q = SQ_FREE; my_first = hd[SQ_FREE]; }
            else if (wv < p1) { my_q = SQ_CMP; my_first = hd[SQ_CMP] + ((wv - p0) << 6); }
            else if (wv < p2) { my_q = SQ_LOC; my_first = hd[SQ_LOC] + ((wv - p1) << 6); }
            else if (wv < p3) { my_q = SQ_STEP; my_first = hd[SQ_STEP] + ((wv - p2) << 6); }
            else { my_q = SQ_BEGIN; my_first = hd[SQ_BEGIN] + ((wv - p3) << 6); }
        } else {
            uint32_t j = wv - p4;
            const uint32_t r_cmp = cn[SQ_CMP] & 63u, r_loc = cn[SQ_LOC] & 63u, r_step = cn[SQ_STEP] & 63u, r_beg = cn[SQ_BEGIN] & 63u;
            bool got = false;
            if (r_free) { if (j == 0) { my_q = SQ_FREE; my_n = r_free; my_first = hd[SQ_FREE]; got = true; } else j--; }
            if (!got && r_cmp) { if (j == 0) { my_q = SQ_CMP; my_n = r_cmp; my_first = hd[SQ_CMP] + (cn[SQ_CMP] & ~63u); got = true; } else j--; }
            if (!got && r_loc) { if (j == 0) { my_q = SQ_LOC; my_n = r_loc; my_first = hd[SQ_LOC] + (cn[SQ_LOC] & ~63u); got = true; } else j--; }
            if (!got && r_step) { if (j == 0) { my_q = SQ_STEP; my_n = r_step; my_first = hd[SQ_STEP] + (cn[SQ_STEP] & ~63u); got = true; } else j--; }
            if (!got && r_beg) { if (j == 0) { my_q = SQ_BEGIN; my_n = r_beg; my_first = hd[SQ_BEGIN] + (cn[SQ_BEGIN] & ~63u); got = true; } else j--; }
        }
        if (my_n == 0) continue;
        wtrips++;
#pragma unroll
        for (int k = 0; k < SQ_NQ; k++) if (k == my_q) { q_trips[k]++; q_lanes[k] += my_n; }
        const bool act = (uint32_t)lane < my_n;
        uint32_t slot = 0;
        if (act) slot = q[(size_t)my_q * QCAP + ((my_first + (uint32_t)lane) & SM)];
        if (lane == 0) atomicAdd(&ctl[my_q], my_n);
        int nq = SQ_FREE;

        if (my_q == SQ_FREE) {
            unsigned int base = 0;
            if (lane == 0) base = atomicAdd(next_read, my_n);
            base = sq_rfl(base);
            const uint32_t avail = base < (unsigned int)n_reads ? (unsigned int)n_reads - base : 0u;
            const uint32_t take = avail < my_n ? avail : my_n;
            if (take < my_n && lane == 0) ctl[10] = 1u;
            if (act && (uint32_t)lane < take) {
                const uint32_t r = base + (uint32_t)lane;
                tab[wave * 64 + lane] = (uint16_t)slot;
                st[slot * 3] = make_uint4(r, (uint32_t)rlen[r], 0u, 0u);
                nq = SQ_BEGIN;
            }
            asm volatile("s_waitcnt lgkmcnt(0)" ::: "memory");
            const uint32_t total = take * (uint32_t)W;
            const uint32_t *src = enc + (size_t)base * W;
            for (uint32_t i0 = 0; i0 < total; i0 += 256u) {
                uint32_t v[4];
#pragma unroll
                for (int k = 0; k < 4; k++) { const uint32_t i = i0 + (uint32_t)(k * 64 + lane); v[k] = i < total ? src[i] : 0u; }
#pragma unroll
                for (int k = 0; k < 4; k++) {
                    const uint32_t i = i0 + (uint32_t)(k * 64 + lane);
                    if (i < total) { const uint32_t rk = (i * w_magic) >> 20; rd[(size_t)(i - rk * (uint32_t)W) * NSLOT + tab[wave * 64 + rk]] = v[k]; }
                }
            }
        } else if (my_q == SQ_BEGIN) nq = sq_trip<SQ_BEGIN>(env, act, slot, c, max_trips);
        else if (my_q == SQ_STEP) nq = sq_trip<SQ_STEP>(env, act, slot, c, max_trips);
        else if (my_q == SQ_CMP) nq = sq_trip<SQ_CMP>(env, act, slot, c, max_trips);
        else nq = sq_trip<SQ_LOC>(env, act, slot, c, max_trips);
        {
            unsigned long long m[SQ_NQ];
#pragma unroll
            for (int k = 0; k < SQ_NQ; k++) m[k] = __ballot(act && nq == k);
            uint32_t mine = 0;
            unsigned long long mq = 0;
#pragma unroll
            for (int k = 0; k < SQ_NQ; k++) { if (lane == k) mine = (uint32_t)__popcll(m[k]); if (nq == k) mq = m[k]; }
            uint32_t base = 0;
            if (lane < SQ_NQ && mine) base = atomicAdd(&ctl[5 + lane], mine);
            base = (uint32_t)__shfl((int)base, nq, 64);
            if (act) q[(size_t)nq * QCAP + ((base + (uint32_t)__popcll(mq & ((1ull << lane) - 1ull))) & SM)] = (uint16_t)slot;
        }
    }
    atomicMax(d_ctr_stripe(ctr) + CTR_MAXTRIPS, (unsigned long long)max_trips);
    if (tid == 0) atomicAdd(d_ctr_stripe(ctr) + CTR_SQ_PHASES, (unsigned long long)n_phases);
    if (lane == 0) {
        atomicMax(d_ctr_stripe(ctr) + CTR_WTRIPS_MAX, (unsigned long long)wtrips); atomicAdd(d_ctr_stripe(ctr) + CTR_WTRIPS_SUM, (unsigned long long)wtrips);
#pragma unroll
        for (int k = 0; k < SQ_NQ; k++) if (q_trips[k]) { atomicAdd(d_ctr_stripe(ctr) + CTR_SQ_TRIPS + k, (unsigned long long)q_trips[k]); atomicAdd(d_ctr_stripe(ctr) + CTR_SQ_LANES + k, (unsigned long long)q_lanes[k]); }
    }
    d_wave_add(ctr + CTR_STEPS, c.steps);
    d_wave_add(ctr + CTR_BLOCKS, c.blocks);
    d_wave_add(ctr + CTR_STEPS_ACT, c.steps_act);
    d_wave_add(ctr + CTR_BLOCKS_ACT, c.blocks_act);
    d_wave_add(ctr + CTR_KTAB, c.ktab);
    d_wave_add(ctr + CTR_LF, c.lf_ref);
    d_wave_add(ctr + CTR_LF_ACT, c.lf_act);
    d_wave_add(ctr + CTR_DIRECT, c.n_direct);
}


#define SQF_FULL 0x8000u
#define SQF_LAP  0x4000u
#define SQF_MAX_LOOKS (1u << 24)

__host__ __device__ inline size_t sqf_lds_bytes(int nslot_lg, int W, int n_waves)
{
    const size_t n = (size_t)1 << nslot_lg;
    return n * 32 + n * 4 * (size_t)W + n * 2 * SQ_NQ + (size_t)n_waves * 64 * 2 + 32 * 4;
}

__device__ __forceinline__ uint32_t sqf_ld32(const uint32_t *p) { return __hip_atomic_load(p, __ATOMIC_RELAXED, __HIP_MEMORY_SCOPE_WORKGROUP); }
__device__ __forceinline__ uint32_t sqf_ld16(const uint16_t *p) { return (uint32_t)__hip_atomic_load(p, __ATOMIC_RELAXED, __HIP_MEMORY_SCOPE_WORKGROUP); }
__device__ __forceinline__ void sqf_st16(uint16_t *p, uint32_t v) { __hip_atomic_store(p, (uint16_t)v, __ATOMIC_RELAXED, __HIP_MEMORY_SCOPE_WORKGROUP); }

struct SqfDelta { uint32_t steps, blocks, lf_ref, max_trips;
#ifdef DG_SQF_PROF
    unsigned long long t, prof[12];
#endif
};
#ifdef DG_SQF_PROF
#define SQF_T(dl, i) do { const unsigned long long n_ = __builtin_amdgcn_s_memtime(); (dl).prof[i] += n_ - (dl).t; (dl).t = n_; } while (0)
#define SQF_TW(dl, i) do { asm volatile("s_waitcnt vmcnt(0) lgkmcnt(0)" ::: "memory"); SQF_T(dl, i); } while (0)
#else
#define SQF_T(dl, i)
#define SQF_TW(dl, i)
#endif

#define SQF_MULTI_MAX 4
template <int MODE, bool MULTI = false>
__device__ __forceinline__ int sqf_trip(const SqEnv &e, const bool act, const uint32_t slot, SqfDelta &dl)
{
    const DIndex &ix = e.ix;
    const int NSLOT = e.NSLOT, W2 = e.W2;
    uint32_t *rd = e.rd; uint4 *st = e.st;
    int nq = SQ_FREE;
    SeedCtr c = {0, 0, 0, 0, 0, 0, 0, 0};
    uint4 A = make_uint4(0, 0, 0, 0), B = A;
    if (act) { A = st[slot * 2]; if (MODE != SQ_BEGIN) B = st[slot * 2 + 1]; }
    const int r = (int)A.x, len = (int)(A.y & 0x3FFu), end_pos = len - 13;
    int pos = (int)((A.y >> 10) & 0x3FFu), nh = (int)(A.z & 31u);
    uint32_t nsearch = (A.z >> 5) & 31u, trips = (A.z >> 10) & 0xFFu, ns = A.w & 0xFFFFFu;
    Search s;
    s.mode = MODE; s.hit_len = 0; s.located = false;
    s.start = pos; s.p = (int)(A.y >> 20); s.ref_steps = A.z >> 18; s.ref_blocks = A.w >> 20;
    s.x0 = s.x1 = s.lk = 0; s.x2 = 1; s.tpos = 0; s.lsteps = 0;
    if (MODE == SQ_STEP) { s.x0 = d_u64(B.x, B.w & 0xFFu); s.x1 = d_u64(B.y, (B.w >> 8) & 0xFFu); s.x2 = d_u64(B.z, (B.w >> 16) & 0xFFu); }
    else if (MODE == SQ_LOC) { s.lk = d_u64(B.x, B.y & 0xFFu); s.lsteps = B.y >> 8; }
    else if (MODE == SQ_CMP) { s.tpos = (int64_t)d_u64(B.x, B.y & 0xFFu); s.lsteps = B.y >> 8; s.lk = (uint64_t)B.z << 40; }
    uint32_t nx = MODE == SQ_LOC ? B.z : 1u;
    auto rb = [&](int w) -> uint32_t { const int wc = w < W2 ? w : W2 - 1; const uint32_t v = rd[(size_t)wc * NSLOT + slot]; return w < W2 ? v : 0u; };
    auto rm = [&](int w) -> uint32_t { const int wc = w < W2 ? w : W2 - 1; const uint32_t v = rd[(size_t)(W2 + wc) * NSLOT + slot]; return w < W2 ? v : 0xFFFFFFFFu; };
    bool live = act, finished = false, beginning = false;
    TripData t; t.aux = T_NONE;
    TripAddr ta = {nullptr, nullptr, nullptr, nullptr};
    uint32_t mt = 0;
    if (act) {
        trips = trips < 255u ? trips + 1u : trips;
        if (MODE == SQ_BEGIN) {
            while (pos < end_pos && d_at(rm, pos)) pos++;
            if (pos >= end_pos) finished = true;
            else if (nsearch >= SEED_BAIL || trips >= (uint32_t)e.bail_trips) {
                DHeavy hv; hv.read = (uint32_t)r; hv.pos = pos; hv.nh = nh; hv.ns = ns;
                e.heavy[atomicAdd(e.n_heavy, 1u)] = hv;
                mt = trips;
                live = false;
            } else { nsearch++; beginning = true; d_begin_issue(ix, e.K, rb, rm, pos, s, c, ta, t); }
        } else if (!(MODE == SQ_LOC && MULTI)) d_trip_issue<MODE == SQ_STEP ? TM_STEP : (MODE == SQ_CMP ? TM_CMP : TM_LOC)>(ix, rm, len, e.direct, s, c, ta, t);
    }
    SQF_TW(dl, 2);
    if (!(MODE == SQ_LOC && MULTI)) d_trip_load(ta, t);
    SQF_TW(dl, 3);
    auto between = [&]() {
        if (e.direct && s.mode == 1 && s.x2 == 1) { s.mode = 3; s.lk = s.x0; s.lsteps = 0; nx = 1u; }
        if (s.mode == 1 && (s.p >= len || d_at(rm, s.p))) d_search_end(e.pr, s);
        if (s.mode == 1 && s.x2 <= (uint64_t)e.multi) { s.mode = 3; s.lk = s.x0; s.lsteps = 0; nx = (uint32_t)s.x2; }
    };
    auto multi = [&](const bool go) {
        uint2 sa[SQF_MULTI_MAX];
#pragma unroll
        for (int i = 0; i < SQF_MULTI_MAX; i++) sa[i] = make_uint2(0u, 0u);
        const bool have_pos = s.mode == 2;
        if (have_pos) { nx = 1u; sa[0] = make_uint2((uint32_t)s.lk, (uint32_t)(s.lk >> 32)); }
        const uint2 *sap = (const uint2 *)ix.sa_dense + (have_pos ? 0ull : s.lk);
#pragma unroll
        for (int i = 0; i < SQF_MULTI_MAX; i++) if (go && !have_pos && (uint32_t)i < nx) sa[i] = sap[i];
        SQF_TW(dl, 3);
        const uint32_t *pw = (const uint32_t *)ix.pac;
        uint4 s16[SQF_MULTI_MAX]; uint2 s8[SQF_MULTI_MAX]; uint32_t sh[SQF_MULTI_MAX]; int tnv[SQF_MULTI_MAX];
#pragma unroll
        for (int i = 0; i < SQF_MULTI_MAX; i++) {
            s16[i] = make_uint4(0u, 0u, 0u, 0u); s8[i] = make_uint2(0u, 0u); sh[i] = 0u; tnv[i] = 0;
            if (go && (uint32_t)i < nx) {
                const Text64At at = d_text64_at(ix, (int64_t)(d_u64(sa[i].x, sa[i].y & 0xFFu) - 1ull) + (s.p - s.start));
                s16[i] = *(const uint4_a4 *)(pw + at.word); s8[i] = *(const uint2_a4 *)(pw + at.word + 4); sh[i] = at.sh; tnv[i] = at.nv;
            }
        }
        SQF_TW(dl, 5);
        if (go) {
            const int w = s.p >> 4;
            const uint32_t o = (uint32_t)((s.p & 15) << 1);
            const uint32_t b0 = rb(w), b1 = rb(w + 1), b2 = rb(w + 2), b3 = rb(w + 3), b4 = rb(w + 4);
            const uint32_t m0 = rm(w), m1 = rm(w + 1), m2 = rm(w + 2), m3 = rm(w + 3), m4 = rm(w + 4);
            const uint32_t R0 = __funnelshift_l(b1, b0, o), R1 = __funnelshift_l(b2, b1, o), R2 = __funnelshift_l(b3, b2, o), R3 = __funnelshift_l(b4, b3, o);
            const uint32_t N0 = __funnelshift_l(m1, m0, o), N1 = __funnelshift_l(m2, m1, o), N2 = __funnelshift_l(m3, m2, o), N3 = __funnelshift_l(m4, m3, o);
            constexpr int chunk = 64;
            const int in_read = len - s.p < chunk ? len - s.p : chunk;
            int jj[SQF_MULTI_MAX];
#pragma unroll
            for (int i = 0; i < SQF_MULTI_MAX; i++) {
                jj[i] = -1;
                if ((uint32_t)i < nx) {
                    Text64At at; at.word = 0; at.sh = sh[i]; at.nv = tnv[i]; at.mirror = false; at.slow = false;
                    const Text64 x = d_text64_words(ix, at, s16[i].x, s16[i].y, s16[i].z, s16[i].w, s8[i].x);
                    const int nv = x.nv;
                    const uint32_t T0 = x.T0, T1 = x.T1, T2 = x.T2, T3 = x.T3;
                    const int lim = in_read < nv ? in_read : nv;
                    auto tail = [&](int k) -> uint32_t { const int rem = lim - 16 * k; return rem >= 16 ? 0u : (rem <= 0 ? 0xFFFFFFFFu : 0xFFFFFFFFu >> (2 * rem)); };
                    const uint32_t e0 = (R0 ^ T0) | N0 | tail(0), e1 = (R1 ^ T1) | N1 | tail(1), e2 = (R2 ^ T2) | N2 | tail(2), e3 = (R3 ^ T3) | N3 | tail(3);
                    jj[i] = e0 ? __clz((int)e0) >> 1 : e1 ? 16 + (__clz((int)e1) >> 1) : e2 ? 32 + (__clz((int)e2) >> 1) : e3 ? 48 + (__clz((int)e3) >> 1) : 64;
                }
            }
            int j = -1, first = 0, cnt = 0;
#pragma unroll
            for (int i = 0; i < SQF_MULTI_MAX; i++) if (jj[i] > j) j = jj[i];
#pragma unroll
            for (int i = SQF_MULTI_MAX - 1; i >= 0; i--) if (jj[i] == j) { first = i; cnt++; }
            uint2 se = sa[0];
#pragma unroll
            for (int i = 1; i < SQF_MULTI_MAX; i++) if (first == i) se = sa[i];
            s.ref_steps += (uint32_t)j; s.ref_blocks += (uint32_t)j;
            s.p += j;
            c.n_direct++;
            if (cnt == 1) {
                const uint64_t en = d_u64(se.x, se.y);
                s.tpos = (int64_t)((en & 0xFFFFFFFFFFull) - 1ull); s.lk = en; s.lsteps = 0; s.x2 = 1; s.mode = 2;
            } else { s.x0 = s.lk + (uint64_t)first; s.x2 = (uint64_t)cnt; s.lk = s.x0; nx = (uint32_t)cnt; s.mode = j < chunk ? 1 : 3; }
            if (j < chunk) {
                const uint32_t nsel = j < 16 ? N0 : j < 32 ? N1 : j < 48 ? N2 : N3;
                if (j < in_read && !((nsel >> (30 - ((j & 15) << 1))) & 1u)) { s.ref_steps++; s.ref_blocks++; }
                d_search_end(e.pr, s);
            }
        }
    };
    if (MODE == SQ_LOC && MULTI) multi(live);
    else if (live) {
        if (MODE == SQ_BEGIN) { if (beginning) d_begin_finish(ix, e.K, rb, s, c, t); }
        else if (t.aux != T_NONE) d_trip_finish<MODE == SQ_STEP ? TM_STEP : (MODE == SQ_CMP ? TM_CMP : TM_LOC)>(ix, e.pr, rb, rm, len, s, c, t);
        between();
    }
    SQF_TW(dl, 4);
    if (MODE == SQ_BEGIN && MULTI) multi(live && (s.mode == 2 || s.mode == 3));
    else if (MODE == SQ_BEGIN || MODE == SQ_LOC) {
        constexpr int M2 = TM_CMP;
        const bool go = live && ((M2 & TM_STEP) && s.mode == 1 || (M2 & TM_CMP) && s.mode == 2);
        TripData t2; t2.aux = T_NONE;
        TripAddr ta2 = {nullptr, nullptr, nullptr, nullptr};
        if (go) d_trip_issue<M2>(ix, rm, len, e.direct, s, c, ta2, t2);
        d_trip_load(ta2, t2);
        SQF_TW(dl, 5);
        if (go && t2.aux != T_NONE) { d_trip_finish<M2>(ix, e.pr, rb, rm, len, s, c, t2); between(); }
    }
    if (live) {
        if (!finished && s.mode == 0) {
            if (s.hit_len) {
                if (nh < e.H) {
                    DHit h; h.rPos = (uint16_t)s.start; h.len = (uint16_t)s.hit_len;
                    if (s.located) { h.x0 = (uint64_t)s.tpos; h.freq = 1u | 0x80000000u; c.lf_ref += s.lsteps + (uint32_t)(s.lk >> 40); }
                    else { h.x0 = s.x0; h.freq = (uint32_t)s.x2; }
                    e.hits[(size_t)r * e.H + nh] = h;
                }
                nh++; ns += (uint32_t)s.x2;
                pos = s.start + s.hit_len;
            } else pos = s.start + 1;
            dl.steps += s.ref_steps; dl.blocks += s.ref_blocks;
            while (pos < end_pos && d_at(rm, pos)) pos++;
            if (pos >= end_pos) finished = true;
            s.ref_steps = s.ref_blocks = 0;
        }
        if (finished) { e.nhits[r] = (uint32_t)nh; e.nseeds[r] = ns; mt = trips; }
        else {
            nq = s.mode;
            A.y = (uint32_t)len | ((uint32_t)pos << 10) | ((uint32_t)(s.mode ? s.p : 0) << 20);
            A.z = (uint32_t)nh | (nsearch << 5) | (trips << 10) | (s.ref_steps << 18); A.w = ns | (s.ref_blocks << 20);
            st[slot * 2] = A;
            if (s.mode == 1) st[slot * 2 + 1] = make_uint4((uint32_t)s.x0, (uint32_t)s.x1, (uint32_t)s.x2, (uint32_t)(s.x0 >> 32) | ((uint32_t)(s.x1 >> 32) << 8) | ((uint32_t)(s.x2 >> 32) << 16));
            else if (s.mode == 3) st[slot * 2 + 1] = make_uint4((uint32_t)s.lk, (uint32_t)((s.lk >> 32) & 0xFFu) | (s.lsteps << 8), nx, 0u);
            else if (s.mode == 2) st[slot * 2 + 1] = make_uint4((uint32_t)s.tpos, (uint32_t)(((uint64_t)s.tpos >> 32) & 0xFFu) | (s.lsteps << 8), (uint32_t)(s.lk >> 40), 0u);
        }
    }
    dl.lf_ref += (uint32_t)c.lf_ref; dl.max_trips = mt > dl.max_trips ? mt : dl.max_trips;
    SQF_TW(dl, 6);
    return nq;
}

__global__ void __launch_bounds__(512)
k_seed_qf(const DIndex ix, const DParams pr, const uint32_t *__restrict__ enc, const uint16_t *__restrict__ rlen, int n_reads, int W, int H, int nslot_lg,
          DHit *__restrict__ hits, uint32_t *__restrict__ nhits, uint32_t *__restrict__ nseeds, unsigned int *next_read,
          DHeavy *__restrict__ heavy, unsigned int *n_heavy, unsigned long long *ctr, int bail_trips, int partial_min, int multi, int *err, int drain_bail)
{
    const unsigned long long t_wave0 = wall_clock64();
    extern __shared__ uint4 sq_sh[];
    const int NSLOT = 1 << nslot_lg;
    const int QCAP = NSLOT, QLG = nslot_lg;
    const uint32_t SM = (uint32_t)QCAP - 1u;
    const int n_waves = (int)(blockDim.x >> 6);
    uint4 *st = sq_sh;
    uint32_t *rd = (uint32_t *)(st + 2 * (size_t)NSLOT);
    uint16_t *q = (uint16_t *)(rd + (size_t)W * NSLOT);
    uint16_t *tab = q + (size_t)SQ_NQ * QCAP;
    uint32_t *ctl = (uint32_t *)(tab + (size_t)n_waves * 64);
    const int tid = threadIdx.x, lane = tid & 63;
    const int wave = (int)sq_rfl((uint32_t)(tid >> 6));
    const int W2 = W >> 1;
    const int K = ix.ktab ? ix.ktab_k : 0;
    const bool direct = ix.sa_dense != nullptr;
    const uint32_t w_magic = ((1u << 20) + (uint32_t)W - 1u) / (uint32_t)W;
    const SqEnv env = { ix, pr, st, rd, NSLOT, W2, K, H, bail_trips, direct, (direct && ix.sa_dense_intv == 1) ? multi : 0, hits, nhits, nseeds, heavy, n_heavy };
    SqEnv env_drain = env; env_drain.bail_trips = drain_bail;
    unsigned long long acc_steps = 0, acc_blocks = 0, acc_lf = 0;
    uint32_t max_trips = 0, wtrips = 0;

    for (int i = tid; i < SQ_NQ * QCAP; i += (int)blockDim.x) q[i] = (uint16_t)(i >= SQ_FREE * QCAP ? (SQF_FULL | (uint32_t)(i - SQ_FREE * QCAP)) : SQF_LAP);
    if (tid < 32) ctl[tid] = tid == 8 + SQ_FREE ? (uint32_t)NSLOT : 0u;
    __syncthreads();

    uint32_t looks = 0, lazy = 0;
    bool running = true;
#ifdef DG_SQF_PROF
    SqfDelta pf; for (int i = 0; i < 12; i++) pf.prof[i] = 0; pf.t = __builtin_amdgcn_s_memtime();
    const unsigned long long pf_t0 = pf.t;
#endif
    while (running) {
        const uint32_t cw = sqf_ld32(&ctl[lane & 15]);
        uint32_t hd[SQ_NQ], cn[SQ_NQ];
#pragma unroll
        for (int k = 0; k < SQ_NQ; k++) {
            hd[k] = (uint32_t)__builtin_amdgcn_readlane((int)cw, k);
            cn[k] = (uint32_t)__builtin_amdgcn_readlane((int)cw, 8 + k) - hd[k];
            if (cn[k] > (uint32_t)NSLOT) cn[k] = 0u;
        }
        const bool ex = __builtin_amdgcn_readlane((int)cw, 5) != 0;
        int my_q = -1;
        uint32_t my_n = 0;
        if (!ex && cn[SQ_FREE] >= 64u) { my_q = SQ_FREE; my_n = 64u; }
        else if (cn[SQ_CMP] >= 64u) { my_q = SQ_CMP; my_n = 64u; }
        else if (cn[SQ_LOC] >= 64u) { my_q = SQ_LOC; my_n = 64u; }
        else if (cn[SQ_STEP] >= 64u) { my_q = SQ_STEP; my_n = 64u; }
        else if (cn[SQ_BEGIN] >= 64u) { my_q = SQ_BEGIN; my_n = 64u; }
        else {
            uint32_t best = ex ? 0u : cn[SQ_FREE];
            my_q = best ? SQ_FREE : -1;
            if (cn[SQ_CMP] > best) { best = cn[SQ_CMP]; my_q = SQ_CMP; }
            if (cn[SQ_LOC] > best) { best = cn[SQ_LOC]; my_q = SQ_LOC; }
            if (cn[SQ_STEP] > best) { best = cn[SQ_STEP]; my_q = SQ_STEP; }
            if (cn[SQ_BEGIN] > best) { best = cn[SQ_BEGIN]; my_q = SQ_BEGIN; }
            my_n = best;
            if (best == 0u || (best < (uint32_t)partial_min && lazy < 2u)) { my_q = -1; if (best) lazy++; }
        }
        uint32_t got = 0;
        if (my_q >= 0 && lane == 0) got = atomicCAS(&ctl[my_q], hd[my_q], hd[my_q] + my_n) == hd[my_q] ? 1u : 0u;
        const bool go = my_q >= 0 && sq_rfl(got) != 0u;
        SQF_TW(pf, 0);
        if (go) {
            lazy = 0;
            const uint32_t my_first = hd[my_q];
            wtrips++;
            if (lane == 0) { atomicAdd(&ctl[16 + my_q], 1u); atomicAdd(&ctl[24 + my_q], my_n); }
            const bool act = (uint32_t)lane < my_n;
            uint32_t slot = 0;
            if (act) {
                const uint32_t a = my_first + (uint32_t)lane, want = SQF_FULL | (((a >> QLG) & 1u) ? SQF_LAP : 0u);
                uint16_t *ep = q + (size_t)my_q * QCAP + (a & SM);
                uint32_t e = sqf_ld16(ep);
                while ((e & (SQF_FULL | SQF_LAP)) != want) { __builtin_amdgcn_s_sleep(1); e = sqf_ld16(ep); }
                slot = e & 0x3FFFu;
                sqf_st16(ep, want & SQF_LAP);
            }
            __builtin_amdgcn_fence(__ATOMIC_ACQUIRE, "workgroup", "local");
            int nq = SQ_FREE;
            SqfDelta dl = {0u, 0u, 0u, 0u};
#ifdef DG_SQF_PROF
            SQF_TW(pf, 1);
            for (int i = 0; i < 12; i++) dl.prof[i] = 0;
            dl.t = pf.t;
#endif

            if (my_q == SQ_FREE) {
                unsigned int base = 0;
                if (lane == 0) base = atomicAdd(next_read, my_n);
                base = sq_rfl(base);
                SQF_TW(dl, 10);
                const uint32_t avail = base < (unsigned int)n_reads ? (unsigned int)n_reads - base : 0u;
                const uint32_t take = avail < my_n ? avail : my_n;
                if (take < my_n && lane == 0) __hip_atomic_store(&ctl[5], 1u, __ATOMIC_RELAXED, __HIP_MEMORY_SCOPE_WORKGROUP);
                const bool mine_r = act && (uint32_t)lane < take;
                const uint32_t total = take * (uint32_t)W;
                const uint32_t *src = enc + (size_t)base * W;
                uint32_t my_len = 0;
                if (mine_r) { my_len = (uint32_t)rlen[base + (uint32_t)lane]; tab[wave * 64 + lane] = (uint16_t)slot; nq = SQ_BEGIN; }
                for (uint32_t i0 = 0; i0 < total; i0 += 1024u) {
                    uint32_t v[16];
#ifdef DG_SQF_PROF
                    { const uint32_t i = i0 + (uint32_t)lane; v[0] = i < total ? src[i] : 0u; }
                    SQF_TW(dl, 11);
#pragma unroll
                    for (int k = 1; k < 16; k++) { const uint32_t i = i0 + (uint32_t)(k * 64 + lane); v[k] = i < total ? src[i] : 0u; }
                    SQF_TW(dl, 9);
#else
#pragma unroll
                    for (int k = 0; k < 16; k++) { const uint32_t i = i0 + (uint32_t)(k * 64 + lane); v[k] = i < total ? src[i] : 0u; }
#endif
                    if (i0 == 0u) {
                        if (mine_r) st[slot * 2] = make_uint4(base + (uint32_t)lane, my_len, 0u, 0u);
                        asm volatile("s_waitcnt lgkmcnt(0)" ::: "memory");
                    }
#pragma unroll
                    for (int k = 0; k < 16; k++) {
                        const uint32_t i = i0 + (uint32_t)(k * 64 + lane);
                        if (i < total) { const uint32_t rk = (i * w_magic) >> 20; rd[(size_t)(i - rk * (uint32_t)W) * NSLOT + tab[wave * 64 + rk]] = v[k]; }
                    }
                }
            } else if (my_q == SQ_BEGIN) { const SqEnv &eb = ex ? env_drain : env; if (env.multi) nq = sqf_trip<SQ_BEGIN, true>(eb, act, slot, dl); else nq = sqf_trip<SQ_BEGIN>(eb, act, slot, dl); }
            else if (my_q == SQ_STEP) nq = sqf_trip<SQ_STEP>(env, act, slot, dl);
            else if (my_q == SQ_CMP) nq = sqf_trip<SQ_CMP>(env, act, slot, dl);
            else if (env.multi) nq = sqf_trip<SQ_LOC, true>(env, act, slot, dl);
            else nq = sqf_trip<SQ_LOC>(env, act, slot, dl);
#ifdef DG_SQF_PROF
            if (my_q == SQ_FREE) SQF_TW(dl, 9);
            for (int i = 0; i < 12; i++) pf.prof[i] += dl.prof[i];
            pf.t = dl.t;
#endif
            acc_steps += dl.steps; acc_blocks += dl.blocks; acc_lf += dl.lf_ref; max_trips = dl.max_trips > max_trips ? dl.max_trips : max_trips;
            __builtin_amdgcn_fence(__ATOMIC_RELEASE, "workgroup", "local");
            unsigned long long m[SQ_NQ];
#pragma unroll
            for (int k = 0; k < SQ_NQ; k++) m[k] = __ballot(act && nq == k);
            uint32_t mine = 0;
            unsigned long long mq = 0;
#pragma unroll
            for (int k = 0; k < SQ_NQ; k++) { if (lane == k) mine = (uint32_t)__popcll(m[k]); if (nq == k) mq = m[k]; }
            uint32_t base = 0;
            if (lane < SQ_NQ && mine) base = atomicAdd(&ctl[8 + lane], mine);
            base = (uint32_t)__shfl((int)base, nq, 64);
            if (act) {
                const uint32_t a = base + (uint32_t)__popcll(mq & ((1ull << lane) - 1ull));
                const uint32_t lap = ((a >> QLG) & 1u) ? SQF_LAP : 0u;
                uint16_t *ep = q + (size_t)nq * QCAP + (a & SM);
                while (sqf_ld16(ep) != (lap ^ SQF_LAP)) __builtin_amdgcn_s_sleep(1);
                sqf_st16(ep, SQF_FULL | lap | slot);
            }
            SQF_TW(pf, 7);
        } else if (my_q < 0) {
            if (ex && cn[SQ_FREE] == (uint32_t)NSLOT) running = false;
            else {
                if (lane == 0) atomicAdd(&ctl[21], 1u);
                __builtin_amdgcn_s_sleep(32);
            }
            SQF_T(pf, 8);
        }
        if (++looks > SQF_MAX_LOOKS) { if (lane == 0) atomicMax(err, DG_E_SEEDQ); running = false; }
    }
#ifdef DG_SQF_PROF
    if (lane == 0 && (blockIdx.x % 97u) == 0u && (wave & 3) == 0)
        printf("sqf wg %u wave %d: total %llu trips %u looks %u | look %llu pop %llu issue %llu mem1 %llu fin1 %llu mem2 %llu fin2+store %llu push %llu idle %llu refill %llu refill_atomic %llu refill_loads %llu\n", blockIdx.x, wave,
               __builtin_amdgcn_s_memtime() - pf_t0, wtrips, looks, pf.prof[0], pf.prof[1], pf.prof[2], pf.prof[3], pf.prof[4], pf.prof[5], pf.prof[6], pf.prof[7], pf.prof[8], pf.prof[9], pf.prof[10], pf.prof[11]);
#endif
    atomicMax(d_ctr_stripe(ctr) + CTR_MAXTRIPS, (unsigned long long)max_trips);
    if (lane == 0) { atomicMax(d_ctr_stripe(ctr) + CTR_WTRIPS_MAX, (unsigned long long)wtrips); atomicAdd(d_ctr_stripe(ctr) + CTR_WTRIPS_SUM, (unsigned long long)wtrips); }
    d_wave_add(ctr + CTR_STEPS, acc_steps);
    d_wave_add(ctr + CTR_BLOCKS, acc_blocks);
    d_wave_add(ctr + CTR_LF, acc_lf);
    d_wave_resident(ctr, CTR_WT_SEEDQF, t_wave0);
    __syncthreads();
    if (tid < SQ_NQ) {
        atomicAdd(d_ctr_stripe(ctr) + CTR_SQ_TRIPS + tid, (unsigned long long)ctl[16 + tid]); atomicAdd(d_ctr_stripe(ctr) + CTR_SQ_LANES + tid, (unsigned long long)ctl[24 + tid]);
        if (tid == 0) atomicAdd(d_ctr_stripe(ctr) + CTR_SQ_PHASES, (unsigned long long)ctl[21]);
    }
}
```

Baseline: 1219.

## Add two-slots-per-lane seed queue kernel variant for memory-level parallelism

Measured after the change: 1189. 2.5% lower.

```diff
diff --git a/dart_amd/csrc/dg_api.hip b/dart_amd/csrc/dg_api.hip
--- a/dart_amd/csrc/dg_api.hip
+++ b/dart_amd/csrc/dg_api.hip
@@ -143,7 +143,7 @@
     bool want_full = true, full_valid = false;
     int n_cu = 256, runs_of_last_batch = 0, attempt_no = 0;
     int env_seed_waves = 4, env_bail_trips = 0 , env_report_bpc = 8, env_no_fast = 0, env_seed_legacy = 0, env_seed_slots_lg = 0, env_seed_wgs = 0, env_blocking_sync = 0;
-    int env_seed_phases = 0, env_seed_wg_waves = 4, env_seed_partial = 32, env_seed_multi = 4;
+    int env_seed_phases = 0, env_seed_wg_waves = 4, env_seed_partial = 32, env_seed_multi = 4, env_seed_lane_slots = SQF_LANE_SLOTS;
     bool seed_qf_used = false;
     int env_scan_mask = 7;
     int env_chain_bpc = 8, env_seedh_bpc = 8, env_reseed_pct = 100;
@@ -166,6 +166,7 @@
     c->env_report_bpc = geti("DG_REPORT_BPC", 8); c->env_no_fast = geti("DG_NO_FAST_PAIR", 0);
     c->env_scan_budget = geti("DG_SCAN_POLL_BUDGET", 0); c->env_scan_mask = geti("DG_SCAN_POLL_SCANS", 7);
     c->env_seed_phases = geti("DG_SEED_PHASES", 0); c->env_seed_wg_waves = geti("DG_SEED_WG_WAVES", 4); c->env_seed_partial = geti("DG_SEED_PARTIAL_MIN", 32);
+    c->env_seed_lane_slots = geti("DG_SEED_LANE_SLOTS", SQF_LANE_SLOTS); if (c->env_seed_lane_slots != 1 && c->env_seed_lane_slots != 2) c->env_seed_lane_slots = SQF_LANE_SLOTS;
     c->env_copy_stream = geti("DG_COPY_STREAM", 1);
     c->env_chain_bpc = std::max(1, geti("DG_CHAIN_BPC", 8)); c->env_seedh_bpc = std::max(1, geti("DG_SEEDH_BPC", 8)); c->env_reseed_pct = std::max(10, geti("DG_RESEED_PCT", 100));
     c->env_rs_chunk = geti("DG_RS_CHUNK", RS_CHUNK_DIAGS); c->env_rs_chunk = std::min(1 << 24, std::max(RS_SUPER, c->env_rs_chunk / RS_SUPER * RS_SUPER));
@@ -1374,7 +1375,7 @@
 
 #define DG_MAX_DEVICES 64
 static std::mutex g_lds_mu;
-static size_t g_lds_set[2][DG_MAX_DEVICES];
+static size_t g_lds_set[3][DG_MAX_DEVICES];
 static hipError_t raise_dynamic_lds(const void *fn, int which, int device, size_t lds)
 {
     std::lock_guard<std::mutex> lk(g_lds_mu);
@@ -1407,7 +1408,8 @@
         while (lg > 6 && sqf_lds_bytes(lg, W, nw) > (size_t)156 * 1024) lg--;
         if (c->env_seed_slots_lg == 0) while (lg > 6 && sqf_lds_bytes(lg, W, nw) > (size_t)80 * 1024) lg--;
         const size_t lds = sqf_lds_bytes(lg, W, nw);
-        if ((e = raise_dynamic_lds((const void *)k_seed_qf, 0, c->device, lds)) != hipSuccess) return e;
+        const bool two = c->env_seed_lane_slots == 2;
+        if ((e = raise_dynamic_lds(two ? (const void *)k_seed_qf2 : (const void *)k_seed_qf, two ? 2 : 0, c->device, lds)) != hipSuccess) return e;
         unsigned per_cu = (unsigned)(((size_t)160 * 1024) / lds);
         if (per_cu * (unsigned)nw > 16u) per_cu = 16u / (unsigned)nw;
         if (per_cu > 2u) per_cu = 2u;
@@ -1417,7 +1419,7 @@
         const unsigned need = (unsigned)(((size_t)n + ((size_t)1 << lg) - 1) >> lg);
         if (wgs > need) wgs = need;
         c->seed_qf_used = true;
-        k_seed_qf<<<wgs, nw * 64, lds, c->stream>>>(c->ix, c->pr, c->enc.p, c->rlen.p, n, W, H, lg, c->hits.p, c->nhits.p, c->nseeds.p, tops + TOP_SEED_NEXT,
+        (two ? k_seed_qf2 : k_seed_qf)<<<wgs, nw * 64, lds, c->stream>>>(c->ix, c->pr, c->enc.p, c->rlen.p, n, W, H, lg, c->hits.p, c->nhits.p, c->nseeds.p, tops + TOP_SEED_NEXT,
                                                     c->seed_heavy.p, tops + TOP_SEED_HEAVY, c->d_ctr, bail_trips, c->env_seed_partial, c->env_seed_multi, c->d_err, bail_trips);
     } else
     if (!c->env_seed_legacy && W <= 62) {
diff --git a/dart_amd/csrc/dg_seedq.h b/dart_amd/csrc/dg_seedq.h
--- a/dart_amd/csrc/dg_seedq.h
+++ b/dart_amd/csrc/dg_seedq.h
@@ -257,80 +257,122 @@
 #endif
 
 #define SQF_MULTI_MAX 4
-template <int MODE, bool MULTI = false>
-__device__ __forceinline__ int sqf_trip(const SqEnv &e, const bool act, const uint32_t slot, SqfDelta &dl)
+#define SQF_LANE_SLOTS 1
+struct SqfRb { const uint32_t *rd; int NSLOT, W2; uint32_t slot;
+    __device__ __forceinline__ uint32_t operator()(int w) const { const int wc = w < W2 ? w : W2 - 1; const uint32_t v = rd[(size_t)wc * NSLOT + slot]; return w < W2 ? v : 0u; } };
+struct SqfRm { const uint32_t *rd; int NSLOT, W2; uint32_t slot;
+    __device__ __forceinline__ uint32_t operator()(int w) const { const int wc = w < W2 ? w : W2 - 1; const uint32_t v = rd[(size_t)(W2 + wc) * NSLOT + slot]; return w < W2 ? v : 0xFFFFFFFFu; } };
+struct SqfSlot {
+    uint32_t slot; SqfRb rb; SqfRm rm;
+    uint4 A;
+    int r, len, end_pos, pos, nh, nq;
+    uint32_t nsearch, trips, ns, nx, mt;
+    Search s;
+    TripData t; TripAddr ta;
+    bool live, finished, beginning, go;
+    uint2 sa[SQF_MULTI_MAX]; uint4 s16[SQF_MULTI_MAX]; uint2 s8[SQF_MULTI_MAX]; uint32_t sh[SQF_MULTI_MAX]; int tnv[SQF_MULTI_MAX];
+    bool have_pos;
+};
+
+template <int MODE, bool MULTI>
+__device__ __forceinline__ void sqf_open(const SqEnv &e, SqfSlot &z, SeedCtr &c, const bool act, const uint32_t slot)
 {
     const DIndex &ix = e.ix;
-    const int NSLOT = e.NSLOT, W2 = e.W2;
-    uint32_t *rd = e.rd; uint4 *st = e.st;
-    int nq = SQ_FREE;
-    SeedCtr c = {0, 0, 0, 0, 0, 0, 0, 0};
+    z.slot = slot; z.rb = SqfRb{e.rd, e.NSLOT, e.W2, slot}; z.rm = SqfRm{e.rd, e.NSLOT, e.W2, slot};
+    z.nq = SQ_FREE;
     uint4 A = make_uint4(0, 0, 0, 0), B = A;
-    if (act) { A = st[slot * 2]; if (MODE != SQ_BEGIN) B = st[slot * 2 + 1]; }
-    const int r = (int)A.x, len = (int)(A.y & 0x3FFu), end_pos = len - 13;
-    int pos = (int)((A.y >> 10) & 0x3FFu), nh = (int)(A.z & 31u);
-    uint32_t nsearch = (A.z >> 5) & 31u, trips = (A.z >> 10) & 0xFFu, ns = A.w & 0xFFFFFu;
-    Search s;
+    if (act) { A = e.st[slot * 2]; if (MODE != SQ_BEGIN) B = e.st[slot * 2 + 1]; }
+    z.A = A;
+    z.r = (int)A.x; z.len = (int)(A.y & 0x3FFu); z.end_pos = z.len - 13;
+    z.pos = (int)((A.y >> 10) & 0x3FFu); z.nh = (int)(A.z & 31u);
+    z.nsearch = (A.z >> 5) & 31u; z.trips = (A.z >> 10) & 0xFFu; z.ns = A.w & 0xFFFFFu;
+    Search &s = z.s;
     s.mode = MODE; s.hit_len = 0; s.located = false;
-    s.start = pos; s.p = (int)(A.y >> 20); s.ref_steps = A.z >> 18; s.ref_blocks = A.w >> 20;
+    s.start = z.pos; s.p = (int)(A.y >> 20); s.ref_steps = A.z >> 18; s.ref_blocks = A.w >> 20;
     s.x0 = s.x1 = s.lk = 0; s.x2 = 1; s.tpos = 0; s.lsteps = 0;
     if (MODE == SQ_STEP) { s.x0 = d_u64(B.x, B.w & 0xFFu); s.x1 = d_u64(B.y, (B.w >> 8) & 0xFFu); s.x2 = d_u64(B.z, (B.w >> 16) & 0xFFu); }
     else if (MODE == SQ_LOC) { s.lk = d_u64(B.x, B.y & 0xFFu); s.lsteps = B.y >> 8; }
     else if (MODE == SQ_CMP) { s.tpos = (int64_t)d_u64(B.x, B.y & 0xFFu); s.lsteps = B.y >> 8; s.lk = (uint64_t)B.z << 40; }
-    uint32_t nx = MODE == SQ_LOC ? B.z : 1u;
-    auto rb = [&](int w) -> uint32_t { const int wc = w < W2 ? w : W2 - 1; const uint32_t v = rd[(size_t)wc * NSLOT + slot]; return w < W2 ? v : 0u; };
-    auto rm = [&](int w) -> uint32_t { const int wc = w < W2 ? w : W2 - 1; const uint32_t v = rd[(size_t)(W2 + wc) * NSLOT + slot]; return w < W2 ? v : 0xFFFFFFFFu; };
-    bool live = act, finished = false, beginning = false;
-    TripData t; t.aux = T_NONE;
-    TripAddr ta = {nullptr, nullptr, nullptr, nullptr};
-    uint32_t mt = 0;
+    z.nx = MODE == SQ_LOC ? B.z : 1u;
+    z.live = act; z.finished = false; z.beginning = false; z.go = false;
+    z.t.aux = T_NONE;
+    z.ta = TripAddr{nullptr, nullptr, nullptr, nullptr};
+    z.mt = 0;
     if (act) {
-        trips = trips < 255u ? trips + 1u : trips;
+        z.trips = z.trips < 255u ? z.trips + 1u : z.trips;
         if (MODE == SQ_BEGIN) {
-            while (pos < end_pos && d_at(rm, pos)) pos++;
-            if (pos >= end_pos) finished = true;
-            else if (nsearch >= SEED_BAIL || trips >= (uint32_t)e.bail_trips) {
-                DHeavy hv; hv.read = (uint32_t)r; hv.pos = pos; hv.nh = nh; hv.ns = ns;
+            while (z.pos < z.end_pos && d_at(z.rm, z.pos)) z.pos++;
+            if (z.pos >= z.end_pos) z.finished = true;
+            else if (z.nsearch >= SEED_BAIL || z.trips >= (uint32_t)e.bail_trips) {
+                DHeavy hv; hv.read = (uint32_t)z.r; hv.pos = z.pos; hv.nh = z.nh; hv.ns = z.ns;
                 e.heavy[atomicAdd(e.n_heavy, 1u)] = hv;
-                mt = trips;
-                live = false;
-            } else { nsearch++; beginning = true; d_begin_issue(ix, e.K, rb, rm, pos, s, c, ta, t); }
-        } else if (!(MODE == SQ_LOC && MULTI)) d_trip_issue<MODE == SQ_STEP ? TM_STEP : (MODE == SQ_CMP ? TM_CMP : TM_LOC)>(ix, rm, len, e.direct, s, c, ta, t);
-    }
-    SQF_TW(dl, 2);
-    if (!(MODE == SQ_LOC && MULTI)) d_trip_load(ta, t);
+                z.mt = z.trips;
+                z.live = false;
+            } else { z.nsearch++; z.beginning = true; d_begin_issue(ix, e.K, z.rb, z.rm, z.pos, s, c, z.ta, z.t); }
+        } else if (!(MODE == SQ_LOC && MULTI)) d_trip_issue<MODE == SQ_STEP ? TM_STEP : (MODE == SQ_CMP ? TM_CMP : TM_LOC)>(ix, z.rm, z.len, e.direct, s, c, z.ta, z.t);
+    }
+}
+
+__device__ __forceinline__ void sqf_between(const SqEnv &e, SqfSlot &z)
+{
+    Search &s = z.s;
+    if (e.direct && s.mode == 1 && s.x2 == 1) { s.mode = 3; s.lk = s.x0; s.lsteps = 0; z.nx = 1u; }
+    if (s.mode == 1 && (s.p >= z.len || d_at(z.rm, s.p))) d_search_end(e.pr, s);
+    if (s.mode == 1 && s.x2 <= (uint64_t)e.multi) { s.mode = 3; s.lk = s.x0; s.lsteps = 0; z.nx = (uint32_t)s.x2; }
+}
+
+template <int NS>
+__device__ __forceinline__ void sqf_multi(const SqEnv &e, SqfSlot (&zz)[NS], SeedCtr (&cc)[NS], SqfDelta &dl)
+{
+    const DIndex &ix = e.ix;
+#pragma unroll
+    for (int k = 0; k < NS; k++) {
+        SqfSlot &z = zz[k]; Search &s = z.s;
+#pragma unroll
+        for (int i = 0; i < SQF_MULTI_MAX; i++) z.sa[i] = make_uint2(0u, 0u);
+        z.have_pos = s.mode == 2;
+        if (z.have_pos) z.nx = 1u;
+        if (NS == 1 && z.have_pos) z.sa[0] = make_uint2((uint32_t)s.lk, (uint32_t)(s.lk >> 32));
+        const uint2 *sap = (const uint2 *)ix.sa_dense + (z.have_pos ? 0ull : s.lk);
+#pragma unroll
+        for (int i = 0; i < SQF_MULTI_MAX; i++) {
+            const bool ld = z.go && !z.have_pos && (uint32_t)i < z.nx;
+            if (NS == 1) { if (ld) z.sa[i] = sap[i]; }
+            else z.sa[i] = ((const uint2 *)ix.sa_dense)[ld ? s.lk + (uint64_t)i : 0ull];
+        }
+        if (NS != 1 && z.have_pos) z.sa[0] = make_uint2((uint32_t)s.lk, (uint32_t)(s.lk >> 32));
+    }
     SQF_TW(dl, 3);
-    auto between = [&]() {
-        if (e.direct && s.mode == 1 && s.x2 == 1) { s.mode = 3; s.lk = s.x0; s.lsteps = 0; nx = 1u; }
-        if (s.mode == 1 && (s.p >= len || d_at(rm, s.p))) d_search_end(e.pr, s);
-        if (s.mode == 1 && s.x2 <= (uint64_t)e.multi) { s.mode = 3; s.lk = s.x0; s.lsteps = 0; nx = (uint32_t)s.x2; }
-    };
-    auto multi = [&](const bool go) {
-        uint2 sa[SQF_MULTI_MAX];
-#pragma unroll
-        for (int i = 0; i < SQF_MULTI_MAX; i++) sa[i] = make_uint2(0u, 0u);
-        const bool have_pos = s.mode == 2;
-        if (have_pos) { nx = 1u; sa[0] = make_uint2((uint32_t)s.lk, (uint32_t)(s.lk >> 32)); }
-        const uint2 *sap = (const uint2 *)ix.sa_dense + (have_pos ? 0ull : s.lk);
-#pragma unroll
-        for (int i = 0; i < SQF_MULTI_MAX; i++) if (go && !have_pos && (uint32_t)i < nx) sa[i] = sap[i];
-        SQF_TW(dl, 3);
-        const uint32_t *pw = (const uint32_t *)ix.pac;
-        uint4 s16[SQF_MULTI_MAX]; uint2 s8[SQF_MULTI_MAX]; uint32_t sh[SQF_MULTI_MAX]; int tnv[SQF_MULTI_MAX];
+    const uint32_t *pw = (const uint32_t *)ix.pac;
+#pragma unroll
+    for (int k = 0; k < NS; k++) {
+        SqfSlot &z = zz[k]; Search &s = z.s;
 #pragma unroll
         for (int i = 0; i < SQF_MULTI_MAX; i++) {
-            s16[i] = make_uint4(0u, 0u, 0u, 0u); s8[i] = make_uint2(0u, 0u); sh[i] = 0u; tnv[i] = 0;
-            if (go && (uint32_t)i < nx) {
-                const Text64At at = d_text64_at(ix, (int64_t)(d_u64(sa[i].x, sa[i].y & 0xFFu) - 1ull) + (s.p - s.start));
-                s16[i] = *(const uint4_a4 *)(pw + at.word); s8[i] = *(const uint2_a4 *)(pw + at.word + 4); sh[i] = at.sh; tnv[i] = at.nv;
-            }
-        }
-        SQF_TW(dl, 5);
-        if (go) {
+            z.s16[i] = make_uint4(0u, 0u, 0u, 0u); z.s8[i] = make_uint2(0u, 0u); z.sh[i] = 0u; z.tnv[i] = 0;
+            const bool ld = z.go && (uint32_t)i < z.nx;
+            if (NS == 1) {
+                if (ld) {
+                    const Text64At at = d_text64_at(ix, (int64_t)(d_u64(z.sa[i].x, z.sa[i].y & 0xFFu) - 1ull) + (s.p - s.start));
+                    z.s16[i] = *(const uint4_a4 *)(pw + at.word); z.s8[i] = *(const uint2_a4 *)(pw + at.word + 4); z.sh[i] = at.sh; z.tnv[i] = at.nv;
+                }
+            } else {
+                const Text64At at = d_text64_at(ix, (int64_t)(d_u64(z.sa[i].x, z.sa[i].y & 0xFFu) - 1ull) + (s.p - s.start));
+                const uint32_t *p = pw + (ld ? at.word : (int64_t)0);
+                z.s16[i] = *(const uint4_a4 *)p; z.s8[i] = *(const uint2_a4 *)(p + 4); z.sh[i] = ld ? at.sh : 0u; z.tnv[i] = ld ? at.nv : 0;
+            }
+        }
+    }
+    SQF_TW(dl, 5);
+#pragma unroll
+    for (int k = 0; k < NS; k++) {
+        SqfSlot &z = zz[k]; Search &s = z.s;
+        if (z.go) {
+            const int len = z.len;
             const int w = s.p >> 4;
             const uint32_t o = (uint32_t)((s.p & 15) << 1);
-            const uint32_t b0 = rb(w), b1 = rb(w + 1), b2 = rb(w + 2), b3 = rb(w + 3), b4 = rb(w + 4);
-            const uint32_t m0 = rm(w), m1 = rm(w + 1), m2 = rm(w + 2), m3 = rm(w + 3), m4 = rm(w + 4);
+            const uint32_t b0 = z.rb(w), b1 = z.rb(w + 1), b2 = z.rb(w + 2), b3 = z.rb(w + 3), b4 = z.rb(w + 4);
+            const uint32_t m0 = z.rm(w), m1 = z.rm(w + 1), m2 = z.rm(w + 2), m3 = z.rm(w + 3), m4 = z.rm(w + 4);
             const uint32_t R0 = __funnelshift_l(b1, b0, o), R1 = __funnelshift_l(b2, b1, o), R2 = __funnelshift_l(b3, b2, o), R3 = __funnelshift_l(b4, b3, o);
             const uint32_t N0 = __funnelshift_l(m1, m0, o), N1 = __funnelshift_l(m2, m1, o), N2 = __funnelshift_l(m3, m2, o), N3 = __funnelshift_l(m4, m3, o);
             constexpr int chunk = 64;
@@ -339,13 +381,13 @@
 #pragma unroll
             for (int i = 0; i < SQF_MULTI_MAX; i++) {
                 jj[i] = -1;
-                if ((uint32_t)i < nx) {
-                    Text64At at; at.word = 0; at.sh = sh[i]; at.nv = tnv[i]; at.mirror = false; at.slow = false;
-                    const Text64 x = d_text64_words(ix, at, s16[i].x, s16[i].y, s16[i].z, s16[i].w, s8[i].x);
+                if ((uint32_t)i < z.nx) {
+                    Text64At at; at.word = 0; at.sh = z.sh[i]; at.nv = z.tnv[i]; at.mirror = false; at.slow = false;
+                    const Text64 x = d_text64_words(ix, at, z.s16[i].x, z.s16[i].y, z.s16[i].z, z.s16[i].w, z.s8[i].x);
                     const int nv = x.nv;
                     const uint32_t T0 = x.T0, T1 = x.T1, T2 = x.T2, T3 = x.T3;
                     const int lim = in_read < nv ? in_read : nv;
-                    auto tail = [&](int k) -> uint32_t { const int rem = lim - 16 * k; return rem >= 16 ? 0u : (rem <= 0 ? 0xFFFFFFFFu : 0xFFFFFFFFu >> (2 * rem)); };
+                    auto tail = [&](int q) -> uint32_t { const int rem = lim - 16 * q; return rem >= 16 ? 0u : (rem <= 0 ? 0xFFFFFFFFu : 0xFFFFFFFFu >> (2 * rem)); };
                     const uint32_t e0 = (R0 ^ T0) | N0 | tail(0), e1 = (R1 ^ T1) | N1 | tail(1), e2 = (R2 ^ T2) | N2 | tail(2), e3 = (R3 ^ T3) | N3 | tail(3);
                     jj[i] = e0 ? __clz((int)e0) >> 1 : e1 ? 16 + (__clz((int)e1) >> 1) : e2 ? 32 + (__clz((int)e2) >> 1) : e3 ? 48 + (__clz((int)e3) >> 1) : 64;
                 }
@@ -355,79 +397,120 @@
             for (int i = 0; i < SQF_MULTI_MAX; i++) if (jj[i] > j) j = jj[i];
 #pragma unroll
             for (int i = SQF_MULTI_MAX - 1; i >= 0; i--) if (jj[i] == j) { first = i; cnt++; }
-            uint2 se = sa[0];
-#pragma unroll
-            for (int i = 1; i < SQF_MULTI_MAX; i++) if (first == i) se = sa[i];
+            uint2 se = z.sa[0];
+#pragma unroll
+            for (int i = 1; i < SQF_MULTI_MAX; i++) if (first == i) se = z.sa[i];
             s.ref_steps += (uint32_t)j; s.ref_blocks += (uint32_t)j;
             s.p += j;
-            c.n_direct++;
+            cc[k].n_direct++;
             if (cnt == 1) {
                 const uint64_t en = d_u64(se.x, se.y);
                 s.tpos = (int64_t)((en & 0xFFFFFFFFFFull) - 1ull); s.lk = en; s.lsteps = 0; s.x2 = 1; s.mode = 2;
-            } else { s.x0 = s.lk + (uint64_t)first; s.x2 = (uint64_t)cnt; s.lk = s.x0; nx = (uint32_t)cnt; s.mode = j < chunk ? 1 : 3; }
+            } else { s.x0 = s.lk + (uint64_t)first; s.x2 = (uint64_t)cnt; s.lk = s.x0; z.nx = (uint32_t)cnt; s.mode = j < chunk ? 1 : 3; }
             if (j < chunk) {
                 const uint32_t nsel = j < 16 ? N0 : j < 32 ? N1 : j < 48 ? N2 : N3;
                 if (j < in_read && !((nsel >> (30 - ((j & 15) << 1))) & 1u)) { s.ref_steps++; s.ref_blocks++; }
                 d_search_end(e.pr, s);
             }
         }
-    };
-    if (MODE == SQ_LOC && MULTI) multi(live);
-    else if (live) {
-        if (MODE == SQ_BEGIN) { if (beginning) d_begin_finish(ix, e.K, rb, s, c, t); }
-        else if (t.aux != T_NONE) d_trip_finish<MODE == SQ_STEP ? TM_STEP : (MODE == SQ_CMP ? TM_CMP : TM_LOC)>(ix, e.pr, rb, rm, len, s, c, t);
-        between();
-    }
-    SQF_TW(dl, 4);
-    if (MODE == SQ_BEGIN && MULTI) multi(live && (s.mode == 2 || s.mode == 3));
-    else if (MODE == SQ_BEGIN || MODE == SQ_LOC) {
-        constexpr int M2 = TM_CMP;
-        const bool go = live && ((M2 & TM_STEP) && s.mode == 1 || (M2 & TM_CMP) && s.mode == 2);
-        TripData t2; t2.aux = T_NONE;
-        TripAddr ta2 = {nullptr, nullptr, nullptr, nullptr};
-        if (go) d_trip_issue<M2>(ix, rm, len, e.direct, s, c, ta2, t2);
-        d_trip_load(ta2, t2);
-        SQF_TW(dl, 5);
-        if (go && t2.aux != T_NONE) { d_trip_finish<M2>(ix, e.pr, rb, rm, len, s, c, t2); between(); }
-    }
-    if (live) {
-        if (!finished && s.mode == 0) {
+    }
+}
+
+__device__ __forceinline__ void sqf_close(const SqEnv &e, SqfSlot &z, SeedCtr &c, SqfDelta &dl)
+{
+    Search &s = z.s;
+    if (z.live) {
+        if (!z.finished && s.mode == 0) {
             if (s.hit_len) {
-                if (nh < e.H) {
+                if (z.nh < e.H) {
                     DHit h; h.rPos = (uint16_t)s.start; h.len = (uint16_t)s.hit_len;
                     if (s.located) { h.x0 = (uint64_t)s.tpos; h.freq = 1u | 0x80000000u; c.lf_ref += s.lsteps + (uint32_t)(s.lk >> 40); }
                     else { h.x0 = s.x0; h.freq = (uint32_t)s.x2; }
-                    e.hits[(size_t)r * e.H + nh] = h;
-                }
-                nh++; ns += (uint32_t)s.x2;
-                pos = s.start + s.hit_len;
-            } else pos = s.start + 1;
+                    e.hits[(size_t)z.r * e.H + z.nh] = h;
+                }
+                z.nh++; z.ns += (uint32_t)s.x2;
+                z.pos = s.start + s.hit_len;
+            } else z.pos = s.start + 1;
             dl.steps += s.ref_steps; dl.blocks += s.ref_blocks;
-            while (pos < end_pos && d_at(rm, pos)) pos++;
-            if (pos >= end_pos) finished = true;
+            while (z.pos < z.end_pos && d_at(z.rm, z.pos)) z.pos++;
+            if (z.pos >= z.end_pos) z.finished = true;
             s.ref_steps = s.ref_blocks = 0;
         }
-        if (finished) { e.nhits[r] = (uint32_t)nh; e.nseeds[r] = ns; mt = trips; }
+        if (z.finished) { e.nhits[z.r] = (uint32_t)z.nh; e.nseeds[z.r] = z.ns; z.mt = z.trips; }
         else {
-            nq = s.mode;
-            A.y = (uint32_t)len | ((uint32_t)pos << 10) | ((uint32_t)(s.mode ? s.p : 0) << 20);
-            A.z = (uint32_t)nh | (nsearch << 5) | (trips << 10) | (s.ref_steps << 18); A.w = ns | (s.ref_blocks << 20);
-            st[slot * 2] = A;
-            if (s.mode == 1) st[slot * 2 + 1] = make_uint4((uint32_t)s.x0, (uint32_t)s.x1, (uint32_t)s.x2, (uint32_t)(s.x0 >> 32) | ((uint32_t)(s.x1 >> 32) << 8) | ((uint32_t)(s.x2 >> 32) << 16));
-            else if (s.mode == 3) st[slot * 2 + 1] = make_uint4((uint32_t)s.lk, (uint32_t)((s.lk >> 32) & 0xFFu) | (s.lsteps << 8), nx, 0u);
-            else if (s.mode == 2) st[slot * 2 + 1] = make_uint4((uint32_t)s.tpos, (uint32_t)(((uint64_t)s.tpos >> 32) & 0xFFu) | (s.lsteps << 8), (uint32_t)(s.lk >> 40), 0u);
-        }
-    }
-    dl.lf_ref += (uint32_t)c.lf_ref; dl.max_trips = mt > dl.max_trips ? mt : dl.max_trips;
+            z.nq = s.mode;
+            uint4 A = z.A;
+            A.y = (uint32_t)z.len | ((uint32_t)z.pos << 10) | ((uint32_t)(s.mode ? s.p : 0) << 20);
+            A.z = (uint32_t)z.nh | (z.nsearch << 5) | (z.trips << 10) | (s.ref_steps << 18); A.w = z.ns | (s.ref_blocks << 20);
+            e.st[z.slot * 2] = A;
+            if (s.mode == 1) e.st[z.slot * 2 + 1] = make_uint4((uint32_t)s.x0, (uint32_t)s.x1, (uint32_t)s.x2, (uint32_t)(s.x0 >> 32) | ((uint32_t)(s.x1 >> 32) << 8) | ((uint32_t)(s.x2 >> 32) << 16));
+            else if (s.mode == 3) e.st[z.slot * 2 + 1] = make_uint4((uint32_t)s.lk, (uint32_t)((s.lk >> 32) & 0xFFu) | (s.lsteps << 8), z.nx, 0u);
+            else if (s.mode == 2) e.st[z.slot * 2 + 1] = make_uint4((uint32_t)s.tpos, (uint32_t)(((uint64_t)s.tpos >> 32) & 0xFFu) | (s.lsteps << 8), (uint32_t)(s.lk >> 40), 0u);
+        }
+    }
+    dl.lf_ref += (uint32_t)c.lf_ref; dl.max_trips = z.mt > dl.max_trips ? z.mt : dl.max_trips;
+}
+
+template <bool P16, bool P8, int NS>
+__device__ __forceinline__ void sqf_load(const DIndex &ix, SqfSlot &z)
+{
+    {
+        if (NS == 1 || !(P16 || P8)) d_trip_load(z.ta, z.t);
+        else {
+            if (P16) z.t.s16 = *(z.ta.p16 ? z.ta.p16 : (const uint4_a4 *)ix.pac);
+            if (P8) z.t.s8 = *(z.ta.p8 ? z.ta.p8 : (const uint2_a4 *)ix.pac);
+        }
+    }
+}
+
+#define SQF_EACH(...) do { _Pragma("unroll") for (int k = 0; k < NS; k++) { SqfSlot &z = zz[k]; SeedCtr &c = cs.c[k]; (void)c; __VA_ARGS__; } } while (0)
+template <int MODE, bool MULTI, int NS>
+__device__ __forceinline__ void sqf_trip(const SqEnv &e, const bool (&act)[NS], const uint32_t (&slot)[NS], int (&nq)[NS], SqfDelta &dl)
+{
+    const DIndex &ix = e.ix;
+    constexpr int TM = MODE == SQ_STEP ? TM_STEP : (MODE == SQ_CMP ? TM_CMP : TM_LOC);
+    SqfSlot zz[NS];
+    struct { SeedCtr c[NS]; } cs;
+    SQF_EACH(c = SeedCtr{0, 0, 0, 0, 0, 0, 0, 0}; sqf_open<MODE, MULTI>(e, z, c, act[k], slot[k]));
+    SQF_TW(dl, 2);
+    if (!(MODE == SQ_LOC && MULTI)) SQF_EACH(sqf_load<MODE == SQ_BEGIN || MODE == SQ_CMP, MODE == SQ_CMP, NS>(ix, z));
+    SQF_TW(dl, 3);
+    if (MODE == SQ_LOC && MULTI) {
+        SQF_EACH(z.go = z.live);
+        sqf_multi<NS>(e, zz, cs.c, dl);
+    } else {
+        SQF_EACH(
+            if (z.live) {
+                if (MODE == SQ_BEGIN) { if (z.beginning) d_begin_finish(ix, e.K, z.rb, z.s, c, z.t); }
+                else if (z.t.aux != T_NONE) d_trip_finish<TM>(ix, e.pr, z.rb, z.rm, z.len, z.s, c, z.t);
+                sqf_between(e, z);
+            });
+    }
+    SQF_TW(dl, 4);
+    if (MODE == SQ_BEGIN && MULTI) {
+        SQF_EACH(z.go = z.live && (z.s.mode == 2 || z.s.mode == 3));
+        sqf_multi<NS>(e, zz, cs.c, dl);
+    } else if (MODE == SQ_BEGIN || MODE == SQ_LOC) {
+        constexpr int M2 = TM_CMP;
+        SQF_EACH(
+            z.go = z.live && ((M2 & TM_STEP) && z.s.mode == 1 || (M2 & TM_CMP) && z.s.mode == 2);
+            z.t.aux = T_NONE;
+            z.ta = TripAddr{nullptr, nullptr, nullptr, nullptr};
+            if (z.go) d_trip_issue<M2>(ix, z.rm, z.len, e.direct, z.s, c, z.ta, z.t));
+        SQF_EACH(sqf_load<true, true, NS>(ix, z));
+        SQF_TW(dl, 5);
+        SQF_EACH(if (z.go && z.t.aux != T_NONE) { d_trip_finish<M2>(ix, e.pr, z.rb, z.rm, z.len, z.s, c, z.t); sqf_between(e, z); });
+    }
+    SQF_EACH(sqf_close(e, z, c, dl); nq[k] = z.nq);
     SQF_TW(dl, 6);
-    return nq;
-}
-
-__global__ void __launch_bounds__(512)
-k_seed_qf(const DIndex ix, const DParams pr, const uint32_t *__restrict__ enc, const uint16_t *__restrict__ rlen, int n_reads, int W, int H, int nslot_lg,
+}
+
+template <int NS>
+__device__ __forceinline__ void sqf_run(const DIndex &ix, const DParams &pr, const uint32_t *__restrict__ enc, const uint16_t *__restrict__ rlen, int n_reads, int W, int H, int nslot_lg,
           DHit *__restrict__ hits, uint32_t *__restrict__ nhits, uint32_t *__restrict__ nseeds, unsigned int *next_read,
           DHeavy *__restrict__ heavy, unsigned int *n_heavy, unsigned long long *ctr, int bail_trips, int partial_min, int multi, int *err, int drain_bail)
 {
+    static_assert(NS == 1 || NS == 2, "one or two slots per lane");
     const unsigned long long t_wave0 = wall_clock64();
     extern __shared__ uint4 sq_sh[];
     const int NSLOT = 1 << nslot_lg;
@@ -475,8 +558,8 @@
         if (!ex && cn[SQ_FREE] >= 64u) { my_q = SQ_FREE; my_n = 64u; }
         else if (cn[SQ_CMP] >= 64u) { my_q = SQ_CMP; my_n = 64u; }
         else if (cn[SQ_LOC] >= 64u) { my_q = SQ_LOC; my_n = 64u; }
-        else if (cn[SQ_STEP] >= 64u) { my_q = SQ_STEP; my_n = 64u; }
-        else if (cn[SQ_BEGIN] >= 64u) { my_q = SQ_BEGIN; my_n = 64u; }
+        else if (cn[SQ_STEP] >= 64u) { my_q = SQ_STEP; my_n = NS == 2 && cn[SQ_STEP] >= 128u ? 128u : 64u; }
+        else if (cn[SQ_BEGIN] >= 64u) { my_q = SQ_BEGIN; my_n = NS == 2 && env.multi && cn[SQ_BEGIN] >= 128u ? 128u : 64u; }
         else {
             uint32_t best = ex ? 0u : cn[SQ_FREE];
             my_q = best ? SQ_FREE : -1;
@@ -496,19 +579,22 @@
             const uint32_t my_first = hd[my_q];
             wtrips++;
             if (lane == 0) { atomicAdd(&ctl[16 + my_q], 1u); atomicAdd(&ctl[24 + my_q], my_n); }
-            const bool act = (uint32_t)lane < my_n;
-            uint32_t slot = 0;
-            if (act) {
-                const uint32_t a = my_first + (uint32_t)lane, want = SQF_FULL | (((a >> QLG) & 1u) ? SQF_LAP : 0u);
-                uint16_t *ep = q + (size_t)my_q * QCAP + (a & SM);
-                uint32_t e = sqf_ld16(ep);
-                while ((e & (SQF_FULL | SQF_LAP)) != want) { __builtin_amdgcn_s_sleep(1); e = sqf_ld16(ep); }
-                slot = e & 0x3FFFu;
-                sqf_st16(ep, want & SQF_LAP);
+            bool act[NS]; uint32_t slot[NS]; int nq[NS];
+#pragma unroll
+            for (int k = 0; k < NS; k++) {
+                act[k] = (uint32_t)(64 * k + lane) < my_n; slot[k] = 0; nq[k] = SQ_FREE;
+                if (act[k]) {
+                    const uint32_t a = my_first + (uint32_t)(64 * k + lane), want = SQF_FULL | (((a >> QLG) & 1u) ? SQF_LAP : 0u);
+                    uint16_t *ep = q + (size_t)my_q * QCAP + (a & SM);
+                    uint32_t e = sqf_ld16(ep);
+                    while ((e & (SQF_FULL | SQF_LAP)) != want) { __builtin_amdgcn_s_sleep(1); e = sqf_ld16(ep); }
+                    slot[k] = e & 0x3FFFu;
+                    sqf_st16(ep, want & SQF_LAP);
+                }
             }
             __builtin_amdgcn_fence(__ATOMIC_ACQUIRE, "workgroup", "local");
-            int nq = SQ_FREE;
             SqfDelta dl = {0u, 0u, 0u, 0u};
+            const bool both = NS == 2 && my_n > 64u;
 #ifdef DG_SQF_PROF
             SQF_TW(pf, 1);
             for (int i = 0; i < 12; i++) dl.prof[i] = 0;
@@ -523,11 +609,11 @@
                 const uint32_t avail = base < (unsigned int)n_reads ? (unsigned int)n_reads - base : 0u;
                 const uint32_t take = avail < my_n ? avail : my_n;
                 if (take < my_n && lane == 0) __hip_atomic_store(&ctl[5], 1u, __ATOMIC_RELAXED, __HIP_MEMORY_SCOPE_WORKGROUP);
-                const bool mine_r = act && (uint32_t)lane < take;
+                const bool mine_r = act[0] && (uint32_t)lane < take;
                 const uint32_t total = take * (uint32_t)W;
                 const uint32_t *src = enc + (size_t)base * W;
                 uint32_t my_len = 0;
-                if (mine_r) { my_len = (uint32_t)rlen[base + (uint32_t)lane]; tab[wave * 64 + lane] = (uint16_t)slot; nq = SQ_BEGIN; }
+                if (mine_r) { my_len = (uint32_t)rlen[base + (uint32_t)lane]; tab[wave * 64 + lane] = (uint16_t)slot[0]; nq[0] = SQ_BEGIN; }
                 for (uint32_t i0 = 0; i0 < total; i0 += 1024u) {
                     uint32_t v[16];
 #ifdef DG_SQF_PROF
@@ -541,7 +627,7 @@
                     for (int k = 0; k < 16; k++) { const uint32_t i = i0 + (uint32_t)(k * 64 + lane); v[k] = i < total ? src[i] : 0u; }
 #endif
                     if (i0 == 0u) {
-                        if (mine_r) st[slot * 2] = make_uint4(base + (uint32_t)lane, my_len, 0u, 0u);
+                        if (mine_r) st[slot[0] * 2] = make_uint4(base + (uint32_t)lane, my_len, 0u, 0u);
                         asm volatile("s_waitcnt lgkmcnt(0)" ::: "memory");
                     }
 #pragma unroll
@@ -550,11 +636,18 @@
                         if (i < total) { const uint32_t rk = (i * w_magic) >> 20; rd[(size_t)(i - rk * (uint32_t)W) * NSLOT + tab[wave * 64 + rk]] = v[k]; }
                     }
                 }
-            } else if (my_q == SQ_BEGIN) { const SqEnv &eb = ex ? env_drain : env; if (env.multi) nq = sqf_trip<SQ_BEGIN, true>(eb, act, slot, dl); else nq = sqf_trip<SQ_BEGIN>(eb, act, slot, dl); }
-            else if (my_q == SQ_STEP) nq = sqf_trip<SQ_STEP>(env, act, slot, dl);
-            else if (my_q == SQ_CMP) nq = sqf_trip<SQ_CMP>(env, act, slot, dl);
-            else if (env.multi) nq = sqf_trip<SQ_LOC, true>(env, act, slot, dl);
-            else nq = sqf_trip<SQ_LOC>(env, act, slot, dl);
+            } else if (both) {
+                if (my_q == SQ_STEP) sqf_trip<SQ_STEP, false, NS>(env, act, slot, nq, dl);
+                else sqf_trip<SQ_BEGIN, true, NS>(ex ? env_drain : env, act, slot, nq, dl);
+            } else {
+                const bool a1[1] = {act[0]}; const uint32_t s1[1] = {slot[0]}; int n1[1] = {SQ_FREE};
+                if (my_q == SQ_BEGIN) { const SqEnv &eb = ex ? env_drain : env; if (env.multi) sqf_trip<SQ_BEGIN, true, 1>(eb, a1, s1, n1, dl); else sqf_trip<SQ_BEGIN, false, 1>(eb, a1, s1, n1, dl); }
+                else if (my_q == SQ_STEP) sqf_trip<SQ_STEP, false, 1>(env, a1, s1, n1, dl);
+                else if (my_q == SQ_CMP) sqf_trip<SQ_CMP, false, 1>(env, a1, s1, n1, dl);
+                else if (env.multi) sqf_trip<SQ_LOC, true, 1>(env, a1, s1, n1, dl);
+                else sqf_trip<SQ_LOC, false, 1>(env, a1, s1, n1, dl);
+                nq[0] = n1[0];
+            }
 #ifdef DG_SQF_PROF
             if (my_q == SQ_FREE) SQF_TW(dl, 9);
             for (int i = 0; i < 12; i++) pf.prof[i] += dl.prof[i];
@@ -562,22 +655,33 @@
 #endif
             acc_steps += dl.steps; acc_blocks += dl.blocks; acc_lf += dl.lf_ref; max_trips = dl.max_trips > max_trips ? dl.max_trips : max_trips;
             __builtin_amdgcn_fence(__ATOMIC_RELEASE, "workgroup", "local");
-            unsigned long long m[SQ_NQ];
-#pragma unroll
-            for (int k = 0; k < SQ_NQ; k++) m[k] = __ballot(act && nq == k);
-            uint32_t mine = 0;
-            unsigned long long mq = 0;
-#pragma unroll
-            for (int k = 0; k < SQ_NQ; k++) { if (lane == k) mine = (uint32_t)__popcll(m[k]); if (nq == k) mq = m[k]; }
+            unsigned long long mq[NS];
+            uint32_t mine = 0, before[NS];
+#pragma unroll
+            for (int j = 0; j < NS; j++) { mq[j] = 0; before[j] = 0; }
+#pragma unroll
+            for (int k = 0; k < SQ_NQ; k++) {
+                uint32_t n_k = 0;
+#pragma unroll
+                for (int j = 0; j < NS; j++) {
+                    const unsigned long long m = __ballot(act[j] && nq[j] == k);
+                    if (nq[j] == k) { mq[j] = m; before[j] = n_k; }
+                    n_k += (uint32_t)__popcll(m);
+                }
+                if (lane == k) mine = n_k;
+            }
             uint32_t base = 0;
             if (lane < SQ_NQ && mine) base = atomicAdd(&ctl[8 + lane], mine);
-            base = (uint32_t)__shfl((int)base, nq, 64);
-            if (act) {
-                const uint32_t a = base + (uint32_t)__popcll(mq & ((1ull << lane) - 1ull));
-                const uint32_t lap = ((a >> QLG) & 1u) ? SQF_LAP : 0u;
-                uint16_t *ep = q + (size_t)nq * QCAP + (a & SM);
-                while (sqf_ld16(ep) != (lap ^ SQF_LAP)) __builtin_amdgcn_s_sleep(1);
-                sqf_st16(ep, SQF_FULL | lap | slot);
+#pragma unroll
+            for (int j = 0; j < NS; j++) {
+                const uint32_t bj = (uint32_t)__shfl((int)base, nq[j], 64);
+                if (act[j]) {
+                    const uint32_t a = bj + before[j] + (uint32_t)__popcll(mq[j] & ((1ull << lane) - 1ull));
+                    const uint32_t lap = ((a >> QLG) & 1u) ? SQF_LAP : 0u;
+                    uint16_t *ep = q + (size_t)nq[j] * QCAP + (a & SM);
+                    while (sqf_ld16(ep) != (lap ^ SQF_LAP)) __builtin_amdgcn_s_sleep(1);
+                    sqf_st16(ep, SQF_FULL | lap | slot[j]);
+                }
             }
             SQF_TW(pf, 7);
         } else if (my_q < 0) {
@@ -607,3 +711,19 @@
         if (tid == 0) atomicAdd(d_ctr_stripe(ctr) + CTR_SQ_PHASES, (unsigned long long)ctl[21]);
     }
 }
+
+__global__ void __launch_bounds__(512)
+k_seed_qf(const DIndex ix, const DParams pr, const uint32_t *__restrict__ enc, const uint16_t *__restrict__ rlen, int n_reads, int W, int H, int nslot_lg,
+          DHit *__restrict__ hits, uint32_t *__restrict__ nhits, uint32_t *__restrict__ nseeds, unsigned int *next_read,
+          DHeavy *__restrict__ heavy, unsigned int *n_heavy, unsigned long long *ctr, int bail_trips, int partial_min, int multi, int *err, int drain_bail)
+{
+    sqf_run<1>(ix, pr, enc, rlen, n_reads, W, H, nslot_lg, hits, nhits, nseeds, next_read, heavy, n_heavy, ctr, bail_trips, partial_min, multi, err, drain_bail);
+}
+
+__global__ void __launch_bounds__(512)
+k_seed_qf2(const DIndex ix, const DParams pr, const uint32_t *__restrict__ enc, const uint16_t *__restrict__ rlen, int n_reads, int W, int H, int nslot_lg,
+           DHit *__restrict__ hits, uint32_t *__restrict__ nhits, uint32_t *__restrict__ nseeds, unsigned int *next_read,
+           DHeavy *__restrict__ heavy, unsigned int *n_heavy, unsigned long long *ctr, int bail_trips, int partial_min, int multi, int *err, int drain_bail)
+{
+    sqf_run<2>(ix, pr, enc, rlen, n_reads, W, H, nslot_lg, hits, nhits, nseeds, next_read, heavy, n_heavy, ctr, bail_trips, partial_min, multi, err, drain_bail);
+}
```
